# NoahVl/Explaining-In-Style-Reproducibility-Study

Measured on AMD Instinct MI355X. Metric: StylEx G+D+enc train-step images/sec @256px, higher is better.
Workload: dtype bf16; 1 GPU; FFHQ-shaped 256x256 StylEx, batch 32/GPU, GAE=2 (noise+encoder micro-steps), GP every 4th step, ResNet-18 classifier; image_size=256, batch_per_gpu=32, start_step=0, gradient_accumulate_every=2, global_batch=32, parallelism=dp1

## Files before the change

### explaining-in-style-reproducibility-study_amd/csrc/conv_igemm.hip

```cpp
#include <hip/hip_runtime.h>
#include <stdint.h>

#include "stylex_internal.h"

typedef float f32x16 __attribute__((ext_vector_type(16)));
typedef short bf16x8 __attribute__((ext_vector_type(8)));

namespace {

constexpr int BK = 32;

typedef __bf16 bf16x2_t __attribute__((ext_vector_type(2)));
typedef float f32x2_t __attribute__((ext_vector_type(2)));
__device__ __forceinline__ unsigned pack_bf16(float lo, float hi) {
    f32x2_t v = {lo, hi};
    bf16x2_t r = __builtin_convertvector(v, bf16x2_t);
    return *reinterpret_cast<unsigned*>(&r);
}
__device__ __forceinline__ unsigned short f2bf(float f) { return (unsigned short)(pack_bf16(f, 0.f) & 0xffffu); }

struct RowPix {
    int b, oh, ow;
    bool valid;
};
// ... 544 lines not shown
#pragma unroll
                for (int i = 0; i < TN_; ++i)
                    av[i] = *reinterpret_cast<const bf16x8*>(a + (wn * TN_ * 32 + i * 32 + li) * LDHA + ks * 16 + lk * 8);
#pragma unroll
                for (int j = 0; j < TC_; ++j)
                    bv[j] = *reinterpret_cast<const bf16x8*>(b + (wc * TC_ * 32 + j * 32 + li) * LDHB + ks * 16 + lk * 8);
#pragma unroll
                for (int i = 0; i < TN_; ++i)
#pragma unroll
                    for (int j = 0; j < TC_; ++j)
                        acc[i][j] = __builtin_amdgcn_mfma_f32_32x32x16_bf16(av[i], bv[j], acc[i][j], 0, 0, 0);
            }
        } else {
            const float* a = As(st) + wn * TN_ * 32 + li;
            const float* b = Bs(st) + wc * TC_ * 32 + li;
#pragma unroll
            for (int ks = 0; ks < BK / 2; ++ks) {
                float av[TN_], bv[TC_];
#pragma unroll
                for (int i = 0; i < TN_; ++i) av[i] = a[(ks * 2 + lk) * LDA + i * 32];
#pragma unroll
                for (int j = 0; j < TC_; ++j) bv[j] = b[(ks * 2 + lk) * LDB + j * 32];
#pragma unroll
                for (int i = 0; i < TN_; ++i)
#pragma unroll
                    for (int j = 0; j < TC_; ++j)
                        acc[i][j] = __builtin_amdgcn_mfma_f32_32x32x2f32(av[i], bv[j], acc[i][j], 0, 0, 0);
            }
        }
    };

    if (nk > 0) {
        load_tile(0);
        store_tile(0);
    }
    __syncthreads();
    for (int kt = 0, st = 0; kt < nk; ++kt, st ^= 1) {
        if (kt + 1 < nk) load_tile(kt + 1);
        compute(st);
        if (kt + 1 < nk) store_tile(st ^ 1);
        __syncthreads();
    }

    const int lj = lane & 31, lh = lane >> 5;
    float* out = p.y + (long)split * p.N * T * p.Ck;
#pragma unroll
    for (int j = 0; j < TC_; ++j) {
        int c = c0 + wc * TC_ * 32 + j * 32 + lj;
        if (c >= p.Ck) continue;
#pragma unroll
        for (int i = 0; i < TN_; ++i)
#pragma unroll
            for (int r = 0; r < 16; ++r) {
                int n = n0 + wn * TN_ * 32 + i * 32 + (r & 3) + 8 * (r >> 2) + 4 * lh;
                if (n < p.N) out[((long)n * T + tap) * p.Ck + c] = acc[i][j][r];
            }
    }
}

__device__ __forceinline__ float wg_out(float sum, float old, float scale, int acc) {
#pragma clang fp contract(off)
    float v = scale * sum;
    asm volatile("" : "+v"(v));
    return acc ? old + v : v;
}

__device__ __forceinline__ void bias_reduce_block(const float* __restrict__ part, float* __restrict__ db, int N, int splits,
                                                  int blk, float scale, int acc) {
    const int w = threadIdx.x >> 6, l = threadIdx.x & 63;
    const int n = blk * 4 + w;
    if (n >= N) return;
    float v = 0.f;
    for (int s = l; s < splits; s += 64) v += part[(long)s * N + n];
#pragma unroll
    for (int off = 32; off > 0; off >>= 1) v += __shfl_down(v, off);
    if (l == 0) db[n] = wg_out(v, acc ? db[n] : 0.f, scale, acc);
}

__global__ __launch_bounds__(256) void wgrad_reduce_kernel(const float* __restrict__ partial, float* dw,
                                                           int N, int C, int T, int splits, int main_blocks,
                                                           const float* __restrict__ bias_part, float* db, float scale, int accum) {
    __shared__ float tile[256 * 9];
    if ((int)blockIdx.x >= main_blocks) {
        bias_reduce_block(bias_part, db, N, splits, blockIdx.x - main_blocks, scale, accum);
        return;
    }
    const long total = (long)N * C * T;
    const long pairs = (long)N * C;
    const long i0 = (long)blockIdx.x * 256;
    const long i = i0 + threadIdx.x;
    if (T == 9) {
        float acc[9];
#pragma unroll
        for (int t = 0; t < 9; ++t) acc[t] = 0.f;
        if (i < pairs) {
            const int c = (int)(i % C);
            const long n = i / C;
            const float* src = partial + (n * 9) * C + c;
            int k = 0;
            for (; k + 4 <= splits; k += 4) {
                float v[4][9];
#pragma unroll
                for (int u = 0; u < 4; ++u)
#pragma unroll
                    for (int t = 0; t < 9; ++t) v[u][t] = src[(long)(k + u) * total + (long)t * C];
#pragma unroll
                for (int u = 0; u < 4; ++u)
#pragma unroll
                    for (int t = 0; t < 9; ++t) acc[t] += v[u][t];
            }
            for (; k < splits; ++k) {
#pragma unroll
                for (int t = 0; t < 9; ++t) acc[t] += src[(long)k * total + (long)t * C];
            }
        }
#pragma unroll
        for (int t = 0; t < 9; ++t) tile[threadIdx.x * 9 + t] = acc[t];
        __syncthreads();
        const long span = min((long)256, pairs - i0) * 9;
#pragma unroll
        for (int j = 0; j < 9; ++j) {
            const int o = j * 256 + threadIdx.x;
            if (o < span) dw[i0 * 9 + o] = wg_out(tile[o], accum ? dw[i0 * 9 + o] : 0.f, scale, accum);
        }
        return;
    }
    if (i >= pairs) return;
    const int c = (int)(i % C);
    const long n = i / C;
    const float* src = partial + (n * T) * C + c;
    float* dst = dw + i * T;
    for (int t = 0; t < T; ++t) {
        float a = 0.f;
        for (int k = 0; k < splits; ++k) a += src[(long)k * total + (long)t * C];
        dst[t] = wg_out(a, accum ? dst[t] : 0.f, scale, accum);
    }
}

template <int PP, int G>
__global__ __launch_bounds__(256) void wgrad_reduce_small_kernel(const float* __restrict__ partial, float* dw,
                                                                 int N, int C, int T, int splits, int main_blocks,
                                                                 const float* __restrict__ bias_part, float* db, float scale, int accum) {
    static_assert(PP * G == 256, "one thread per (pair, slice group)");
    __shared__ float red[G][PP][9];
    if ((int)blockIdx.x >= main_blocks) {
        bias_reduce_block(bias_part, db, N, splits, blockIdx.x - main_blocks, scale, accum);
        return;
    }
    const long total = (long)N * C * T;
    const long pairs = (long)N * C;
    const int p = threadIdx.x % PP, g = threadIdx.x / PP;
    const long i = (long)blockIdx.x * PP + p;
    const bool ok = i < pairs;
    float acc[9];
#pragma unroll
    for (int t = 0; t < 9; ++t) acc[t] = 0.f;
    if (ok) {
        const float* src = partial + ((i / C) * T) * C + (int)(i % C);
        int k = g;
        for (; k + 3 * G < splits; k += 4 * G) {
            float v[4][9];
#pragma unroll
            for (int u = 0; u < 4; ++u)
#pragma unroll
                for (int t = 0; t < 9; ++t)
                    if (t < T) v[u][t] = src[(long)(k + u * G) * total + (long)t * C];
#pragma unroll
            for (int u = 0; u < 4; ++u)
#pragma unroll
                for (int t = 0; t < 9; ++t)
                    if (t < T) acc[t] += v[u][t];
        }
        for (; k < splits; k += G) {
#pragma unroll
            for (int t = 0; t < 9; ++t)
                if (t < T) acc[t] += src[(long)k * total + (long)t * C];
        }
    }
#pragma unroll
    for (int t = 0; t < 9; ++t) red[g][p][t] = acc[t];
    __syncthreads();
    for (int o = threadIdx.x; o < PP * T; o += 256) {
        const int pp = o / T, t = o - pp * T;
        if ((long)blockIdx.x * PP + pp < pairs) {
            float sum = 0.f;
#pragma unroll
            for (int q = 0; q < G; ++q) sum += red[q][pp][t];
            float* d = dw + (long)blockIdx.x * PP * T + o;
            *d = wg_out(sum, accum ? *d : 0.f, scale, accum);
        }
    }
}

struct WgOut {
    float scale;
    int accumulate;
};
static WgOut wg_out_of(const ConvKParams& p) { return WgOut{p.wg_scale != 0.f ? p.wg_scale : 1.f, p.wg_accumulate}; }

static void launch_wgrad_reduce(const float* partial, float* dw, int N, int C, int T, int splits, hipStream_t s, WgOut wo,
                                const float* bias_part = nullptr, float* db = nullptr) {
    const long pairs = (long)N * C;
    const unsigned extra = (bias_part && db) ? (unsigned)((N + 3) / 4) : 0u;
    if (T <= 9 && splits >= 32 && (pairs <= 2048 || (pairs <= 8192 && splits >= 256))) {
        const unsigned mb = (unsigned)((pairs + 7) / 8);
        hipLaunchKernelGGL((wgrad_reduce_small_kernel<8, 32>), dim3(mb + extra), dim3(256), 0, s, partial, dw, N, C, T, splits,
                           (int)mb, bias_part, db, wo.scale, wo.accumulate);
    } else if (T <= 9 && splits >= 16 && pairs <= 16384) {
        const unsigned mb = (unsigned)((pairs + 31) / 32);
        hipLaunchKernelGGL((wgrad_reduce_small_kernel<32, 8>), dim3(mb + extra), dim3(256), 0, s, partial, dw, N, C, T, splits,
                           (int)mb, bias_part, db, wo.scale, wo.accumulate);
    } else {
        const unsigned mb = (unsigned)((pairs + 255) / 256);
        hipLaunchKernelGGL(wgrad_reduce_kernel, dim3(mb + extra), dim3(256), 0, s, partial, dw, N, C, T, splits, (int)mb,
                           bias_part, db, wo.scale, wo.accumulate);
    }
}

template <typename OUT>
__device__ __forceinline__ OUT cvt_out(float v);
template <>
__device__ __forceinline__ float cvt_out<float>(float v) { return v; }
template <>
__device__ __forceinline__ unsigned short cvt_out<unsigned short>(float v) { return f2bf(v); }

template <typename OUT>
__global__ void pack_weight_kernel(const float* __restrict__ w, OUT* __restrict__ wf, OUT* __restrict__ wb, int N,
                                   int C, int T) {
    long total = (long)N * C * T;
// ... 218 lines not shown
    int blocks = (int)(((vec4 ? total / 4 : total) + 255) / 256);
    if (blocks > 2048) blocks = 2048;
    if (vec4)
        hipLaunchKernelGGL(splitk_epilogue_kernel<true>, dim3(blocks), dim3(256), 0, s, p);
    else
        hipLaunchKernelGGL(splitk_epilogue_kernel<false>, dim3(blocks), dim3(256), 0, s, p);
    return (int)hipGetLastError();
}

int stylex_launch_igemm(ConvKParams p, int precision, void* workspace, int64_t workspace_bytes, hipStream_t s) {
    bool vec = igemm_vec_ok(p);
    if (precision == STYLEX_BF16 && !p.transposed) {
        int rc = stylex_launch_rgb(p, s);
        if (rc != STYLEX_NOT_APPLICABLE) return rc;
        rc = stylex_launch_halo(p, s);
        if (rc != STYLEX_NOT_APPLICABLE) return rc;
    }
    if (p.mask || p.gate_mask) return STYLEX_EINVAL;
    p.ksplit = 1;
    p.kt_per_split = 0;
    p.partial = nullptr;
    if (precision == STYLEX_BF16) {
        int rc = stylex_launch_gather(p, workspace, workspace_bytes, s);
        if (rc == 0) return p.ksplit ? launch_splitk_epilogue(p, s) : 0;
        if (rc != STYLEX_NOT_APPLICABLE) return rc;
    }
    if (workspace) {
        int ks, per;
        igemm_splitk_plan(p, vec, precision, &ks, &per);
        if (ks > 1 && workspace_bytes >= (int64_t)ks * p.M * p.N * (int64_t)sizeof(float)) {
            p.ksplit = ks;
            p.kt_per_split = per;
            p.partial = (float*)workspace;
        }
    }
    int rc;
    if (precision == STYLEX_BF16) {
        const int bk = igemm_bk(p, vec, precision);
        if (bk == 64) rc = dispatch_igemm<true, true, 64, true>(p, s);
        else if (bk == 33) rc = dispatch_igemm<true, true, 32, true>(p, s);
        else rc = vec ? dispatch_igemm<true, true, 32>(p, s) : dispatch_igemm<false, true, 32>(p, s);
    } else {
        rc = vec ? dispatch_igemm<true, false, 32>(p, s) : dispatch_igemm<false, false, 32>(p, s);
    }
    if (rc || p.ksplit <= 1) return rc;
    return launch_splitk_epilogue(p, s);
}

void stylex_wgrad_plan(const ConvKParams& p, int* tn, int* tc, int* splits, long* split_len) {
    bool big = p.N > 64 && p.Ck > 64;
    *tn = big ? 2 : 1;
    *tc = big ? 2 : 1;
    int bt = big ? 128 : 64;
    long tiles = (long)((p.N + bt - 1) / bt) * ((p.Ck + bt - 1) / bt) * p.KH * p.KW;
    long want = (1024 + tiles - 1) / tiles;
    long max_by_len = ((long)p.M + 4 * BK - 1) / (4 * BK);
    long sp = want < 1 ? 1 : want;
    if (sp > max_by_len) sp = max_by_len;
    if (sp < 1) sp = 1;
    if (sp > 1024) sp = 1024;
    long len = (((long)p.M + sp - 1) / sp + BK - 1) / BK * BK;
    sp = ((long)p.M + len - 1) / len;
    *splits = (int)sp;
    *split_len = len;
}

int stylex_launch_wgrad(ConvKParams p, float* partial, float* dw_oihw, int precision, hipStream_t s, float* db, int* db_done) {
    if (db_done) *db_done = 0;
    if (precision == STYLEX_BF16 && !p.s2d_c && stylex_wgrad_pipe_applicable(p)) {
        int slices = 0, tps, blocks, bias_done = 0;
        stylex_wgrad_pipe_plan(p, &slices, &tps, &blocks);
        if (db) p.bias_partial = partial + (long)slices * p.N * 9 * p.Ck;
        int rc = stylex_launch_wgrad_pipe(p, partial, s, &slices, &bias_done);
        if (rc != STYLEX_NOT_APPLICABLE) {
            if (rc) return rc;
            const bool with_db = db && bias_done;
            launch_wgrad_reduce(partial, dw_oihw, p.N, p.Ck, 9, slices, s, wg_out_of(p), with_db ? p.bias_partial : nullptr, with_db ? db : nullptr);
            if (with_db && db_done) *db_done = 1;
            return (int)hipGetLastError();
        }
        p.bias_partial = nullptr;
    }
    if (precision == STYLEX_BF16 && stylex_wgrad_tr_applicable(p)) {
        int ts = 0;
        int rc = stylex_launch_wgrad_tr(p, partial, s, &ts);
        if (rc) return rc;
        launch_wgrad_reduce(partial, dw_oihw, p.N, p.Ck, p.KH * p.KW, ts, s, wg_out_of(p));
        return (int)hipGetLastError();
    }
    int tn, tc, splits;
    long split_len;
    stylex_wgrad_plan(p, &tn, &tc, &splits, &split_len);
    p.split_len = split_len;
    p.y = partial;
    int bt = tn == 2 ? 128 : 64;
    int T = p.KH * p.KW;
    int blocks = ((p.N + bt - 1) / bt) * ((p.Ck + bt - 1) / bt) * T * splits;
    bool vec = (p.Ck % 4 == 0) && (p.N % 4 == 0) && ((reinterpret_cast<uintptr_t>(p.a) & 15) == 0) &&
               ((reinterpret_cast<uintptr_t>(p.a2) & 15) == 0) &&
               (!p.a_scale || (reinterpret_cast<uintptr_t>(p.a_scale) & 15) == 0) &&
               (!p.a2_scale || (reinterpret_cast<uintptr_t>(p.a2_scale) & 15) == 0);
    int rc;
    bool bf = precision == STYLEX_BF16;
    if (tn == 2) {
        rc = bf ? (vec ? launch_wgrad<2, 2, true, true>(p, blocks, s) : launch_wgrad<2, 2, false, true>(p, blocks, s))
                : (vec ? launch_wgrad<2, 2, true, false>(p, blocks, s) : launch_wgrad<2, 2, false, false>(p, blocks, s));
    } else {
        rc = bf ? (vec ? launch_wgrad<1, 1, true, true>(p, blocks, s) : launch_wgrad<1, 1, false, true>(p, blocks, s))
                : (vec ? launch_wgrad<1, 1, true, false>(p, blocks, s) : launch_wgrad<1, 1, false, false>(p, blocks, s));
    }
    if (rc) return rc;
    launch_wgrad_reduce(partial, dw_oihw, p.N, p.Ck, T, splits, s, wg_out_of(p));
    return (int)hipGetLastError();
}

int stylex_launch_wgrad_s2d_folded(ConvKParams p, float* partial, float* dw_oihw, hipStream_t s) {
    int slices = 0;
    int rc = stylex_launch_wgrad_pipe(p, partial, s, &slices, nullptr);
    if (rc) return rc == STYLEX_NOT_APPLICABLE ? STYLEX_EINVAL : rc;
    launch_wgrad_reduce(partial, dw_oihw, p.N, p.s2d_c, 9, slices, s, wg_out_of(p));
    return (int)hipGetLastError();
}

int stylex_launch_pack(const float* w, void* wf, void* wb, int N, int C, int T, int dtype, hipStream_t s) {
    long total = (long)N * C * T;
    int blocks = (int)((total + 255) / 256);
    if (blocks > 4096) blocks = 4096;
    if (blocks < 1) blocks = 1;
    if (dtype == STYLEX_BF16)
        hipLaunchKernelGGL(pack_weight_kernel<unsigned short>, dim3(blocks), dim3(256), 0, s, w, (unsigned short*)wf,
                           (unsigned short*)wb, N, C, T);
    else
        hipLaunchKernelGGL(pack_weight_kernel<float>, dim3(blocks), dim3(256), 0, s, w, (float*)wf, (float*)wb, N, C, T);
    return (int)hipGetLastError();
}

int stylex_launch_pack_s2d(const float* w, void* wf, void* wb, int N, int C, hipStream_t s) {
    long total = (long)N * C * 36;
    int blocks = (int)((total + 255) / 256);
    if (blocks > 4096) blocks = 4096;
    hipLaunchKernelGGL(pack_weight_s2d_kernel, dim3(blocks), dim3(256), 0, s, w, (unsigned short*)wf, (unsigned short*)wb, N, C);
    return (int)hipGetLastError();
}

int stylex_launch_fold_s2d(const float* dw2, float* dw, int N, int C, hipStream_t s) {
    long total = (long)N * C * 9;
    int blocks = (int)((total + 255) / 256);
    if (blocks > 4096) blocks = 4096;
    hipLaunchKernelGGL(fold_weight_s2d_kernel, dim3(blocks), dim3(256), 0, s, dw2, dw, N, C);
    return (int)hipGetLastError();
}
```

### explaining-in-style-reproducibility-study_amd/csrc/conv_wgrad_pipe.hip

```cpp
#include <hip/hip_runtime.h>
#include <stdint.h>
#include <stdlib.h>

#include "stylex_internal.h"

typedef float f32x16 __attribute__((ext_vector_type(16)));
typedef short bf16x8 __attribute__((ext_vector_type(8)));
typedef short s16x4 __attribute__((ext_vector_type(4)));

struct StylexWgPipeArgs {
    int total_tiles;
    int tiles_per_split;
    int otiles, c_tiles;
    int tx_count, ty_count;
};

namespace {

typedef StylexWgPipeArgs WgArgs;
typedef __attribute__((address_space(3))) void* lds_void_ptr;

template <int NP64, int TW>
struct WgCfg {
    static constexpr int kTW = TW;
// ... 47 lines not shown

constexpr unsigned WG_ALL_TAPS = 0x1ffu;
constexpr bool wg_kw_used(unsigned mask, int kw) { return ((mask >> kw) | (mask >> (3 + kw)) | (mask >> (6 + kw))) & 1u; }

template <class Cfg, int S, unsigned MASK = WG_ALL_TAPS>
__device__ __forceinline__ void issue_reads(WgOps& o, const int (&xb)[4], int dyb) {
    constexpr int rho = S % (Cfg::RW + 2), pw = S / (Cfg::RW + 2), par = S & 1;
    static_assert(Cfg::HWD % 4 == 2, "swizzle class of a halo pixel");
    constexpr int q0 = (rho * Cfg::HWD + pw * 16 + 0) * 128, q1 = (rho * Cfg::HWD + pw * 16 + 1) * 128,
                  q2 = (rho * Cfg::HWD + pw * 16 + 2) * 128;
    constexpr int m0 = (2 * rho + 0) & 3, m1 = (2 * rho + 1) & 3, m2 = (2 * rho + 2) & 3;
    if constexpr (wg_kw_used(MASK, 0)) {
        tr_read<q0>(o.b[par][0][0], xb[m0]);
        tr_read<q0 + 512>(o.b[par][0][1], xb[m0]);
    }
    if constexpr (wg_kw_used(MASK, 1)) {
        tr_read<q1>(o.b[par][1][0], xb[m1]);
        tr_read<q1 + 512>(o.b[par][1][1], xb[m1]);
    }
    if constexpr (wg_kw_used(MASK, 2)) {
        tr_read<q2>(o.b[par][2][0], xb[m2]);
        tr_read<q2 + 512>(o.b[par][2][1], xb[m2]);
    }
    if constexpr (rho < Cfg::RW) {
        constexpr int qa = (rho * Cfg::kTW + pw * 16) * 128;
        tr_read<qa>(o.a[rho & 3][0], dyb);
        tr_read<qa + 512>(o.a[rho & 3][1], dyb);
    }
}

template <class Cfg, int S>
__device__ __forceinline__ void wait_reads(WgOps& o) {
    constexpr int rho = S % (Cfg::RW + 2), par = S & 1;
    if constexpr (rho < Cfg::RW)
        asm volatile("s_waitcnt lgkmcnt(0)"
                     : "+v"(o.b[par][0][0]), "+v"(o.b[par][0][1]), "+v"(o.b[par][1][0]), "+v"(o.b[par][1][1]),
                       "+v"(o.b[par][2][0]), "+v"(o.b[par][2][1]), "+v"(o.a[rho & 3][0]), "+v"(o.a[rho & 3][1]));
    else
        asm volatile("s_waitcnt lgkmcnt(0)"
                     : "+v"(o.b[par][0][0]), "+v"(o.b[par][0][1]), "+v"(o.b[par][1][0]), "+v"(o.b[par][1][1]),
                       "+v"(o.b[par][2][0]), "+v"(o.b[par][2][1]));
}

template <class Cfg, int S, bool BIAS, unsigned MASK = WG_ALL_TAPS>
__device__ __forceinline__ void step_mfma(f32x16 (&acc)[9], f32x16& accb, const WgOps& o, bool do_bias, const bf16x8& ones) {
    constexpr int rho = S % (Cfg::RW + 2), par = S & 1;
    const bf16x8 b0 = cat8(o.b[par][0][0], o.b[par][0][1]);
    const bf16x8 b1 = cat8(o.b[par][1][0], o.b[par][1][1]);
    const bf16x8 b2 = cat8(o.b[par][2][0], o.b[par][2][1]);
#pragma unroll
    for (int kh = 0; kh < 3; ++kh) {
        const int r = rho - kh;
        if (r >= 0 && r < Cfg::RW) {
            const bf16x8 av = cat8(o.a[r & 3][0], o.a[r & 3][1]);
            if ((MASK >> (kh * 3 + 0)) & 1u) mfma1(acc[kh * 3 + 0], av, b0);
            if ((MASK >> (kh * 3 + 1)) & 1u) mfma1(acc[kh * 3 + 1], av, b1);
            if ((MASK >> (kh * 3 + 2)) & 1u) mfma1(acc[kh * 3 + 2], av, b2);
        }
    }
    if constexpr (BIAS && rho < Cfg::RW) {
        if (do_bias) {
            const bf16x8 av = cat8(o.a[rho & 3][0], o.a[rho & 3][1]);
            mfma1(accb, av, ones);
        }
    }
}

constexpr unsigned WG_OOB = 0x80000000u;

struct WgCursor {
    int t, b, tx, ty;
};

template <int NP64, int TW, bool BIAS, bool S2D = false>
__global__ __launch_bounds__(512, 2) void conv3x3_wgrad_pipe_kernel(ConvKParams p, WgArgs wa) {
    using Cfg = WgCfg<NP64, TW>;
    constexpr int TR = Cfg::TR, HWD = Cfg::HWD, XPX = Cfg::XPX, X_PIECES = Cfg::X_PIECES;
    constexpr int X_STRIDE = Cfg::X_STRIDE, DY_STRIDE = Cfg::DY_STRIDE, DY_BASE = Cfg::DY_BASE;
    constexpr int XS = Cfg::XS, DS = Cfg::DS, NSLOT = Cfg::NSLOT, NSTEP = Cfg::NSTEP, NX = Cfg::NX, ND = Cfg::ND;
    constexpr int XA = Cfg::XA, DA = Cfg::DA, WAITN = Cfg::WAITN;
    static_assert(NSTEP % 2 == 0, "the operand ping-pong restarts at parity 0 every stage");
    static_assert(NSLOT <= 2 * (NSTEP - 1), "at most two DMA pieces per step");
    static_assert(XA <= DA, "issue order inside a stage: the one-ahead stream first");
    static_assert(!(S2D && BIAS), "the space-to-depth path has no bias sums");
    extern __shared__ __attribute__((aligned(16))) char smem[];
    const int tid = threadIdx.x, lane = tid & 63;
    const int wave = __builtin_amdgcn_readfirstlane(tid >> 6);
    const int W = p.Wo, C = p.Ck, N = p.N;

    int bid = blockIdx.x;
    {
        const int nblk = gridDim.x, q = nblk >> 3, rr = nblk & 7, xcd = bid & 7, idx = bid >> 3;
        bid = (xcd < rr ? xcd * (q + 1) : rr * (q + 1) + (xcd - rr) * q) + idx;
    }
    const int split = __builtin_amdgcn_readfirstlane(bid / wa.otiles);
    const int ot = bid - split * wa.otiles;
    const int nt_ = __builtin_amdgcn_readfirstlane(ot / wa.c_tiles);
    const int n0 = nt_ * (64 * NP64), c0 = (ot - nt_ * wa.c_tiles) * 64;
    const int t_begin = split * wa.tiles_per_split;
    const int t_end = min(wa.total_tiles, t_begin + wa.tiles_per_split);
    const int nst = t_end - t_begin;
    if (nst <= 0) return;

    const int cblk = wave & 1, nb4 = wave >> 1;
    const int nhalf = nb4 & 1, hi2 = nb4 >> 1;
    const int dy_wave_off = NP64 == 2 ? hi2 * 16384 : (TW == 32 ? hi2 * 16 * 128 : hi2 * 4 * TW * 128);
    const int x_wave_off = NP64 == 2 ? 0 : (TW == 32 ? hi2 * 16 * 128 : hi2 * 4 * HWD * 128);

    const int i16 = lane & 15, g = lane >> 4;
    const int lane_px = ((g >> 1) * 8 + (i16 >> 2)) * 128 + (g & 1) * 32 + (i16 & 3) * 8;
    int dyb = lane_px + ((nhalf ^ ((i16 >> 3) & 1)) * 64) + dy_wave_off + DY_BASE;
    int xb[4];
#pragma unroll
    for (int m = 0; m < 4; ++m) xb[m] = lane_px + ((cblk ^ (((m + (i16 >> 2)) >> 1) & 1)) * 64) + x_wave_off;

    const int dpx = lane >> 3;
    const unsigned lslot = (unsigned)((lane & 7) ^ (((lane >> 4) & 1) << 2));
    unsigned vxc[XS];
    int xdst[XS];
#pragma unroll
    for (int k = 0; k < XS; ++k) {
        const int piece = wave + 8 * k;
        const int q = piece * 8 + dpx;
        const int row = q / HWD, col = q - row * HWD;
        const bool ok = piece < X_PIECES && q < XPX && c0 + (int)lslot * 8 < C;
        const unsigned edge = (row == 0 ? 1u : 0u) | (row == TR + 1 ? 2u : 0u) | (col == 0 ? 4u : 0u) | (col == TW + 1 ? 8u : 0u);
        vxc[k] = ok ? (((unsigned)(row * W + col) * (unsigned)C + (unsigned)c0 + lslot * 8u) * 2u) | edge : WG_OOB;
        xdst[k] = piece < X_PIECES ? piece * 1024 : -1;
    }
    unsigned vdy[DS];
#pragma unroll
    for (int k = 0; k < DS; ++k) {
        const int piece = wave + 8 * k;
        const int q = (piece & 15) * 8 + dpx;
        const int r = q / TW, col = q - r * TW;
        const int nch = n0 + (piece >> 4) * 64 + (int)lslot * 8;
        vdy[k] = nch < N ? ((unsigned)(r * W + col) * (unsigned)N + (unsigned)nch) * 2u : WG_OOB;
    }
    const int Hs = __builtin_amdgcn_readfirstlane(p.Ho), Ws = __builtin_amdgcn_readfirstlane(p.Wo);
    const int Cs = __builtin_amdgcn_readfirstlane(p.Ck), Ns = __builtin_amdgcn_readfirstlane(p.N);
    const uint64_t xbase = reinterpret_cast<uint64_t>(p.a) - (uint64_t)((long)(Ws + 1) * Cs * 2);
    const uint64_t xbase_u = ((uint64_t)(unsigned)__builtin_amdgcn_readfirstlane((int)(xbase >> 32)) << 32) |
                             (unsigned)__builtin_amdgcn_readfirstlane((int)(xbase & 0xffffffffu));
    const __amdgpu_buffer_rsrc_t rx = __builtin_amdgcn_make_buffer_rsrc(reinterpret_cast<void*>(xbase_u), 0, 0x40000000, 0x00020000);
    const __amdgpu_buffer_rsrc_t rdy = __builtin_amdgcn_make_buffer_rsrc(const_cast<float*>(p.a2), 0, 0x40000000, 0x00020000);

    WgCursor cx, cd;
    {
        const int r1 = __builtin_amdgcn_readfirstlane(t_begin / wa.ty_count);
        const int b1 = __builtin_amdgcn_readfirstlane(r1 / wa.tx_count);
        cx.t = t_begin, cx.ty = t_begin - r1 * wa.ty_count, cx.tx = r1 - b1 * wa.tx_count, cx.b = b1;
        cd = cx;
    }
    auto advance = [&](WgCursor& c) {
        ++c.t;
        if (++c.ty == wa.ty_count) {
            c.ty = 0;
            if (++c.tx == wa.tx_count) c.tx = 0, ++c.b;
        }
    };
    int xslot_dma = 0, dslot_dma = 0;
#define WG_ISSUE_X(K)                                                                                                \
    {                                                                                                                \
        const bool more_ = cx.t < t_end;                                                                             \
        const unsigned soff_ = (unsigned)(((cx.b * Hs + cx.ty * TR) * Ws + cx.tx * TW) * Cs) * 2u;                   \
        const unsigned edge_ = (cx.ty == 0 ? 1u : 0u) | (cx.ty == wa.ty_count - 1 ? 2u : 0u) | (cx.tx == 0 ? 4u : 0u) | \
                               (cx.tx == wa.tx_count - 1 ? 8u : 0u);                                                 \
// ... 86 lines not shown
            WG_STEP(2)                                    \
            WG_STEP(3)                                    \
            WG_STEP(4)                                    \
            if constexpr (NSTEP == 6) {                   \
                WG_LAST(5)                                \
            } else {                                      \
                WG_STEP(5)                                \
                WG_STEP(6)                                \
                WG_STEP(7)                                \
                WG_STEP(8)                                \
                if constexpr (NSTEP == 12) {              \
                    WG_STEP(9)                            \
                    WG_STEP(10)                           \
                    WG_LAST(11)                           \
                } else {                                  \
                    WG_LAST(9)                            \
                }                                         \
            }                                             \
        }                                                 \
    }
    const int sub = S2D ? c0 / p.s2d_c : 0;
    if constexpr (!S2D) {
        WG_LOOP(WG_ALL_TAPS)
    } else {
        if (sub == 0) WG_LOOP(0x010u)
        else if (sub == 1) WG_LOOP(0x018u)
        else if (sub == 2) WG_LOOP(0x012u)
        else WG_LOOP(0x01bu)
    }
#undef WG_LOOP
#undef WG_LAST
#undef WG_STEP
#undef WG_ISSUE
#undef WG_END_DY
#undef WG_END_X
#undef WG_ISSUE_DY
#undef WG_ISSUE_X
    asm volatile("s_waitcnt lgkmcnt(0)" ::: "memory");
    wait_vmcnt<0>();

    asm volatile("s_nop 15\n\ts_nop 15"
                 : "+v"(acc[0]), "+v"(acc[1]), "+v"(acc[2]), "+v"(acc[3]), "+v"(acc[4]), "+v"(acc[5]), "+v"(acc[6]),
                   "+v"(acc[7]), "+v"(acc[8]), "+v"(accb));

    if constexpr (NP64 == 1) {
        float4* cb = reinterpret_cast<float4*>(smem) + (wave & 3) * (5 * 4 * 64) + lane;
#pragma unroll
        for (int round = 0; round < 2; ++round) {
            __syncthreads();
            if (hi2 == 1) {
#pragma unroll
                for (int tt = 0; tt < 5; ++tt) {
                    const int t = round * 5 + tt;
#pragma unroll
                    for (int q = 0; q < 4; ++q) {
                        const f32x16& v = t < 9 ? acc[t < 9 ? t : 0] : accb;
                        cb[(tt * 4 + q) * 64] = make_float4(v[4 * q], v[4 * q + 1], v[4 * q + 2], v[4 * q + 3]);
                    }
                }
            }
            __syncthreads();
            if (hi2 == 0) {
#pragma unroll
                for (int tt = 0; tt < 5; ++tt) {
                    const int t = round * 5 + tt;
#pragma unroll
                    for (int q = 0; q < 4; ++q) {
                        const float4 u = cb[(tt * 4 + q) * 64];
                        f32x16& v = t < 9 ? acc[t < 9 ? t : 0] : accb;
                        v[4 * q] += u.x, v[4 * q + 1] += u.y, v[4 * q + 2] += u.z, v[4 * q + 3] += u.w;
                    }
                }
            }
        }
        if (hi2 == 1) return;
    }

    const int nbase = n0 + (NP64 == 2 ? nb4 : nhalf) * 32;
    const int lj = lane & 31, lh = lane >> 5;
    if constexpr (S2D) {
        const int Co = p.s2d_c, sy = sub >> 1, sx = sub & 1;
        float* outf = p.y + (long)split * N * 9 * Co;
        const int cl = c0 - sub * Co + cblk * 32 + lj;
#pragma unroll
        for (int t2 = 0; t2 < 5; ++t2) {
            if (t2 == 2) continue;
            const int kh2 = t2 / 3, kw2 = t2 % 3;
            if ((kh2 == 0 && sy == 0) || (kw2 == 0 && sx == 0)) continue;
            const int tap = (kh2 == 0 ? 0 : sy + 1) * 3 + (kw2 == 0 ? 0 : sx + 1);
#pragma unroll
            for (int r = 0; r < 16; ++r) {
                const int n = nbase + (r & 3) + 8 * (r >> 2) + 4 * lh;
                outf[((long)n * 9 + tap) * Co + cl] = acc[t2][r];
            }
        }
        return;
    }
    float* out = p.y + (long)split * N * 9 * C;
    const int c = c0 + cblk * 32 + lj;
    if (nbase >= N || c0 + cblk * 32 >= C) return;
    if (do_bias && lj == 0) {
#pragma unroll
        for (int r = 0; r < 16; ++r) p.bias_partial[(long)split * N + nbase + (r & 3) + 8 * (r >> 2) + 4 * lh] = accb[r];
    }
    if (c >= C) return;
    const float xsc = p.a_scale ? p.a_scale[(long)(t_begin / (wa.tx_count * wa.ty_count)) * C + c] : 1.f;
#pragma unroll
    for (int t = 0; t < 9; ++t)
#pragma unroll
        for (int r = 0; r < 16; ++r) {
            const int n = nbase + (r & 3) + 8 * (r >> 2) + 4 * lh;
            out[((long)n * 9 + t) * C + c] = acc[t][r] * xsc;
        }
}

template <int NP64, int TW>
int launch_wg_s2d(const ConvKParams& p, const WgArgs& wa, int blocks, hipStream_t s) {
    using Cfg = WgCfg<NP64, TW>;
    static int attr_state = 0;
    if (attr_state == 0) {
        hipError_t e = hipFuncSetAttribute(reinterpret_cast<const void*>(conv3x3_wgrad_pipe_kernel<NP64, TW, false, true>),
                                           hipFuncAttributeMaxDynamicSharedMemorySize, Cfg::SMEM);
        attr_state = e == hipSuccess ? 1 : -1;
    }
    if (attr_state < 0) return STYLEX_NOT_APPLICABLE;
    stylex_note_kernel("conv3x3_wgrad_pipe_kernel<%d, %d, false, true>", NP64, TW);
    hipLaunchKernelGGL((conv3x3_wgrad_pipe_kernel<NP64, TW, false, true>), dim3(blocks), dim3(512), Cfg::SMEM, s, p, wa);
    return (int)hipGetLastError();
}

template <int NP64, int TW>
int launch_wg(const ConvKParams& p, const WgArgs& wa, int blocks, bool bias, hipStream_t s) {
    using Cfg = WgCfg<NP64, TW>;
    static bool attr_done = false;
    if (!attr_done) {
        hipError_t e = hipFuncSetAttribute(reinterpret_cast<const void*>(conv3x3_wgrad_pipe_kernel<NP64, TW, true>),
                                           hipFuncAttributeMaxDynamicSharedMemorySize, Cfg::SMEM);
        if (e != hipSuccess) return STYLEX_NOT_APPLICABLE;
        e = hipFuncSetAttribute(reinterpret_cast<const void*>(conv3x3_wgrad_pipe_kernel<NP64, TW, false>),
                                hipFuncAttributeMaxDynamicSharedMemorySize, Cfg::SMEM);
        if (e != hipSuccess) return STYLEX_NOT_APPLICABLE;
        attr_done = true;
    }
    stylex_note_kernel("conv3x3_wgrad_pipe_kernel<%d, %d, %s, false>", NP64, TW, bias ? "true" : "false");
    if (bias) hipLaunchKernelGGL((conv3x3_wgrad_pipe_kernel<NP64, TW, true>), dim3(blocks), dim3(512), Cfg::SMEM, s, p, wa);
    else hipLaunchKernelGGL((conv3x3_wgrad_pipe_kernel<NP64, TW, false>), dim3(blocks), dim3(512), Cfg::SMEM, s, p, wa);
    return (int)hipGetLastError();
}

int g_wg_cus = 0;

}

static int wg_np64(const ConvKParams& p) {
    const char* env = getenv("STYLEX_WGRAD_PIPE_NP");
    if (p.N % 128 != 0 || (env && env[0] == '1')) return 1;
    if (env && env[0] == '2') return 2;
    const int tw = p.Wo >= 32 ? 32 : 16;
    const long tiles = (long)p.B * (p.Wo / tw) * (p.Ho / (128 / tw));
    const long otiles2 = (long)(p.N / 128) * ((p.Ck + 63) / 64);
    const long cus = g_wg_cus > 0 ? g_wg_cus : 256;
    const long per_block = tiles * otiles2 / cus;
    static const long thr = getenv("STYLEX_WGRAD_PIPE_NP_THR") ? atol(getenv("STYLEX_WGRAD_PIPE_NP_THR")) : 48;
    return per_block < thr ? 1 : 2;
}

bool stylex_wgrad_pipe_applicable(const ConvKParams& p) {
    const char* env = getenv("STYLEX_WGRAD_PIPE");
    if (env && env[0] == '0') return false;
    if (!p.act_bf16 || p.KH != 3 || p.KW != 3 || p.stride != 1 || p.pad != 1 || p.Hi != p.Ho || p.Wi != p.Wo) return false;
    if (p.a2_scale) return false;
    if (p.s2d_c && (p.Ck != 4 * p.s2d_c || p.s2d_c % 64 != 0 || p.N % 64 != 0 || p.a_scale)) return false;
    if ((p.Ck % 64 != 0 && p.Ck != 32) || (p.N % 64 != 0 && p.N != 32)) return false;
    const int tw = p.Wo >= 32 ? 32 : 16;
    if (p.Wo % tw != 0 || p.Wo < 16) return false;
    const int tr = 128 / tw;
    if (p.Ho % tr != 0) return false;
    if ((reinterpret_cast<uintptr_t>(p.a) & 15) || (reinterpret_cast<uintptr_t>(p.a2) & 15)) return false;
    if (p.a_scale && (reinterpret_cast<uintptr_t>(p.a_scale) & 3)) return false;
    if ((long)p.B * p.Ho * p.Wo * p.Ck * 2 >= (1l << 30) + (1l << 29) || (long)p.B * p.Ho * p.Wo * p.N * 2 >= (1l << 30) + (1l << 29))
        return false;
    return true;
}

void stylex_wgrad_pipe_plan(const ConvKParams& p, int* slices, int* tiles_per_split, int* blocks) {
    if (!g_wg_cus) {
        int dev = 0, n = 0;
        if (hipGetDevice(&dev) == hipSuccess) (void)hipDeviceGetAttribute(&n, hipDeviceAttributeMultiprocessorCount, dev);
        g_wg_cus = n > 0 ? n : 256;
    }
    const int np64 = wg_np64(p);
    const int tw = p.Wo >= 32 ? 32 : 16;
    const int tr = 128 / tw;
    const long tiles_img = (long)(p.Wo / tw) * (p.Ho / tr);
    const long tiles = (long)p.B * tiles_img;
    const long otiles = (long)((p.N + 64 * np64 - 1) / (64 * np64)) * ((p.Ck + 63) / 64);
    long want = g_wg_cus / otiles;
    if (want < 1) want = 1;
    if (want > tiles) want = tiles;
    long tps = (tiles + want - 1) / want;
    if (p.a_scale) {
        if (tps > tiles_img) tps = tiles_img;
        while (tiles_img % tps) --tps;
    }
    const long splits = (tiles + tps - 1) / tps;
    *tiles_per_split = (int)tps;
    *blocks = (int)(splits * otiles);
    *slices = (int)splits;
}

int stylex_launch_wgrad_pipe(ConvKParams p, float* partial, hipStream_t s, int* slices_out, int* bias_done) {
    if (!stylex_wgrad_pipe_applicable(p)) return STYLEX_NOT_APPLICABLE;
    int slices, tps, blocks;
    stylex_wgrad_pipe_plan(p, &slices, &tps, &blocks);
    const int np64 = wg_np64(p);
    const int tw = p.Wo >= 32 ? 32 : 16;
    const int tr = 128 / tw;
    WgArgs wa;
    wa.tx_count = p.Wo / tw;
    wa.ty_count = p.Ho / tr;
    wa.total_tiles = p.B * wa.tx_count * wa.ty_count;
    wa.tiles_per_split = tps;
    wa.c_tiles = (p.Ck + 63) / 64;
    wa.otiles = ((p.N + 64 * np64 - 1) / (64 * np64)) * wa.c_tiles;
    p.y = partial;
    *slices_out = slices;
    if (p.s2d_c) {
        if (bias_done) *bias_done = 0;
        p.bias_partial = nullptr;
        if (np64 == 2) return tw == 32 ? launch_wg_s2d<2, 32>(p, wa, blocks, s) : launch_wg_s2d<2, 16>(p, wa, blocks, s);
        return tw == 32 ? launch_wg_s2d<1, 32>(p, wa, blocks, s) : launch_wg_s2d<1, 16>(p, wa, blocks, s);
    }
    const bool bias = p.bias_partial != nullptr;
    if (bias_done) *bias_done = bias ? 1 : 0;
    if (np64 == 2) return tw == 32 ? launch_wg<2, 32>(p, wa, blocks, bias, s) : launch_wg<2, 16>(p, wa, blocks, bias, s);
    return tw == 32 ? launch_wg<1, 32>(p, wa, blocks, bias, s) : launch_wg<1, 16>(p, wa, blocks, bias, s);
}
```

### explaining-in-style-reproducibility-study_amd/csrc/conv_wgrad_tr.hip

```cpp
#include <hip/hip_runtime.h>
#include <stdint.h>
#include <stdlib.h>

#include "stylex_internal.h"

typedef float f32x16 __attribute__((ext_vector_type(16)));
typedef short bf16x8 __attribute__((ext_vector_type(8)));
typedef short s16x4 __attribute__((ext_vector_type(4)));
typedef __bf16 bf16x2_t __attribute__((ext_vector_type(2)));
typedef float f32x2_t __attribute__((ext_vector_type(2)));

namespace {

__device__ __forceinline__ unsigned pack_bf16(float lo, float hi) {
    f32x2_t v = {lo, hi};
    bf16x2_t r = __builtin_convertvector(v, bf16x2_t);
    return *reinterpret_cast<unsigned*>(&r);
}

typedef __attribute__((address_space(3))) s16x4* lds_s4_ptr;

__device__ __forceinline__ bf16x8 tr_read8(const char* base, int byte_off) {
    s16x4 lo = __builtin_amdgcn_ds_read_tr16_b64_v4i16((lds_s4_ptr)(base + byte_off));
    s16x4 hi = __builtin_amdgcn_ds_read_tr16_b64_v4i16((lds_s4_ptr)(base + byte_off + 4 * 64));
// ... 25 lines not shown
    const int N = p.N, C = p.Ck;
    const int n_tiles = (N + BNn - 1) / BNn, c_tiles = C8 ? 1 : (C + BC - 1) / BC;
    const int per_split = n_tiles * c_tiles * Teff;

    const int bid = blockIdx.x;
    const int tile = bid % per_split, split = bid / per_split;
    const int tap = tile % Teff;
    const int n0 = ((tile / Teff) / c_tiles) * BNn;
    const int c0 = ((tile / Teff) % c_tiles) * BC;
    const int kh = tap / p.KW, kw = tap - kh * p.KW;

    const int m_begin = (int)((long)split * p.split_len);
    const int m_end = (int)min((long)p.M, (long)m_begin + p.split_len);
    const int nk = (m_end - m_begin + BKP - 1) / BKP;
    const int hw = p.Ho * p.Wo;
    const bool pow2 = (hw & (hw - 1)) == 0 && (p.Wo & (p.Wo - 1)) == 0;
    const int sh_hw = __builtin_ctz((unsigned)hw), sh_w = __builtin_ctz((unsigned)p.Wo);

    constexpr int A_SLOTS = BNn / 8, B_SLOTS = BC / 8;
    constexpr int A_PER = BKP * A_SLOTS / 256, B_PER = BKP * B_SLOTS / 256;
    uint4 ra[A_PER], rb[B_PER];
    const unsigned short* dy = reinterpret_cast<const unsigned short*>(p.a2);
    const unsigned short* xs = reinterpret_cast<const unsigned short*>(p.a);

    auto scaled = [&](uint4 v, const float* sc) -> uint4 {
        float4 a0 = *reinterpret_cast<const float4*>(sc), a1 = *reinterpret_cast<const float4*>(sc + 4);
        float4 f0 = act_unpack4(make_uint2(v.x, v.y)), f1 = act_unpack4(make_uint2(v.z, v.w));
        v.x = pack_bf16(f0.x * a0.x, f0.y * a0.y); v.y = pack_bf16(f0.z * a0.z, f0.w * a0.w);
        v.z = pack_bf16(f1.x * a1.x, f1.y * a1.y); v.w = pack_bf16(f1.z * a1.z, f1.w * a1.w);
        return v;
    };

    auto load_tile = [&](int kt) {
        const int mb = m_begin + kt * BKP;
#pragma unroll
        for (int j = 0; j < A_PER; ++j) {
            const int idx = tid + 256 * j;
            const int pr = idx / A_SLOTS, q = idx % A_SLOTS;
            const int m = mb + pr;
            const int n = n0 + q * 8;
            uint4 v = make_uint4(0u, 0u, 0u, 0u);
            if (m < m_end && n < N) {
                v = *reinterpret_cast<const uint4*>(dy + (long)m * N + n);
                if (p.a2_scale) v = scaled(v, p.a2_scale + (long)(pow2 ? (unsigned)m >> sh_hw : (unsigned)m / (unsigned)hw) * N + n);
            }
            ra[j] = v;
        }
#pragma unroll
        for (int j = 0; j < B_PER; ++j) {
            const int idx = tid + 256 * j;
            const int pr = idx / B_SLOTS, q = idx % B_SLOTS;
            const int m = mb + pr;
            int c, th, tw;
            bool ok = m < m_end;
            if (C8) {
                c = 0;
                th = q / p.KW;
                tw = q - th * p.KW;
                ok = ok && q < T;
            } else {
                c = c0 + q * 8;
                th = kh;
                tw = kw;
                ok = ok && c < C;
            }
            uint4 v = make_uint4(0u, 0u, 0u, 0u);
            if (ok) {
                int b, oh;
                if (pow2) {
                    b = (int)((unsigned)m >> sh_hw);
                    oh = (int)(((unsigned)m & (unsigned)(hw - 1)) >> sh_w);
                } else {
                    b = (int)((unsigned)m / (unsigned)hw);
                    oh = (int)((unsigned)(m - b * hw) / (unsigned)p.Wo);
                }
                const int r = m - b * hw;
                const int ow = r - oh * p.Wo;
                const int ih = oh * p.stride + th - p.pad, iw = ow * p.stride + tw - p.pad;
                if (ih >= 0 && ih < p.Hi && iw >= 0 && iw < p.Wi) {
                    v = *reinterpret_cast<const uint4*>(xs + (((long)b * p.Hi + ih) * p.Wi + iw) * C + c);
                    if (p.a_scale) v = scaled(v, p.a_scale + (long)b * C + c);
                }
            }
            rb[j] = v;
        }
    };

    auto store_tile = [&](int st) {
        char* base = smem + st * STAGE;
#pragma unroll
        for (int j = 0; j < A_PER; ++j) {
            const int idx = tid + 256 * j;
            const int pr = idx / A_SLOTS, q = idx % A_SLOTS;
            *reinterpret_cast<uint4*>(base + (q >> 2) * PANEL + pr * 64 + (q & 3) * 16) = ra[j];
        }
#pragma unroll
        for (int j = 0; j < B_PER; ++j) {
            const int idx = tid + 256 * j;
            const int pr = idx / B_SLOTS, q = idx % B_SLOTS;
            *reinterpret_cast<uint4*>(base + (NPA + (q >> 2)) * PANEL + pr * 64 + (q & 3) * 16) = rb[j];
        }
    };

    f32x16 acc[TN_][TC_];
#pragma unroll
    for (int i = 0; i < TN_; ++i)
#pragma unroll
        for (int j = 0; j < TC_; ++j)
#pragma unroll
            for (int e = 0; e < 16; ++e) acc[i][j][e] = 0.f;

    const int i16 = lane & 15, g = lane >> 4;
    const int lane_off = ((g >> 1) * 8 + (i16 >> 2)) * 64 + ((g & 1) * 16 + (i16 & 3) * 4) * 2;

    auto compute = [&](int st) {
        const char* a_base = smem + st * STAGE + (wn * TN_) * PANEL + lane_off;
        const char* b_base = smem + st * STAGE + (NPA + wc * TC_) * PANEL + lane_off;
#pragma unroll
        for (int ks = 0; ks < BKP / 16; ++ks) {
            bf16x8 av[TN_], bv[TC_];
#pragma unroll
            for (int i = 0; i < TN_; ++i) av[i] = tr_read8(a_base + i * PANEL, ks * 16 * 64);
#pragma unroll
            for (int j = 0; j < TC_; ++j) bv[j] = tr_read8(b_base + j * PANEL, ks * 16 * 64);
#pragma unroll
            for (int i = 0; i < TN_; ++i)
#pragma unroll
                for (int j = 0; j < TC_; ++j)
                    acc[i][j] = __builtin_amdgcn_mfma_f32_32x32x16_bf16(av[i], bv[j], acc[i][j], 0, 0, 0);
        }
    };

    if (nk > 0) {
        load_tile(0);
        store_tile(0);
    }
    __syncthreads();
    for (int kt = 0, st = 0; kt < nk; ++kt, st ^= 1) {
        if (kt + 1 < nk) load_tile(kt + 1);
        compute(st);
        if (kt + 1 < nk) store_tile(st ^ 1);
        __syncthreads();
    }

    const int lj = lane & 31, lh = lane >> 5;
    float* out = p.y + (long)split * N * T * C;
#pragma unroll
    for (int j = 0; j < TC_; ++j) {
        const int cj = c0 + (wc * TC_ + j) * 32 + lj;
        if (C8 ? (cj >= T * 8) : (cj >= C)) continue;
#pragma unroll
        for (int i = 0; i < TN_; ++i)
#pragma unroll
            for (int r = 0; r < 16; ++r) {
                const int n = n0 + (wn * TN_ + i) * 32 + (r & 3) + 8 * (r >> 2) + 4 * lh;
                if (n < N) out[C8 ? ((long)n * T * 8 + cj) : (((long)n * T + tap) * C + cj)] = acc[i][j][r];
            }
    }
}

constexpr int DSTAGES = 4, DPIECES = 4;
constexpr int DSTAGE_BYTES = 8 * PANEL;

struct TrOps {
    s16x4 a[2];
    s16x4 b[2][2];
};
template <int OFF>
__device__ __forceinline__ void tr_asm(s16x4& dst, int addr) {
    asm volatile("ds_read_b64_tr_b16 %0, %1 offset:%2" : "=v"(dst) : "v"(addr), "n"(OFF));
}
template <int KS>
__device__ __forceinline__ void tr_issue(TrOps& o, int a_addr, int b_addr) {
    tr_asm<KS * 16 * 64>(o.a[0], a_addr);
    tr_asm<KS * 16 * 64 + 4 * 64>(o.a[1], a_addr);
    tr_asm<KS * 16 * 64>(o.b[0][0], b_addr);
    tr_asm<KS * 16 * 64 + 4 * 64>(o.b[0][1], b_addr);
    tr_asm<PANEL + KS * 16 * 64>(o.b[1][0], b_addr);
    tr_asm<PANEL + KS * 16 * 64 + 4 * 64>(o.b[1][1], b_addr);
}
template <int N>
__device__ __forceinline__ void tr_wait(TrOps& o) {
    asm volatile("s_waitcnt lgkmcnt(%6)"
                 : "+v"(o.a[0]), "+v"(o.a[1]), "+v"(o.b[0][0]), "+v"(o.b[0][1]), "+v"(o.b[1][0]), "+v"(o.b[1][1])
                 : "n"(N));
}
__device__ __forceinline__ bf16x8 cat8(s16x4 lo, s16x4 hi) {
    bf16x8 r;
    r[0] = lo[0]; r[1] = lo[1]; r[2] = lo[2]; r[3] = lo[3];
    r[4] = hi[0]; r[5] = hi[1]; r[6] = hi[2]; r[7] = hi[3];
    return r;
}

__global__ __launch_bounds__(512, 1) void conv_wgrad_tr_dma_kernel(ConvKParams p) {
    extern __shared__ __attribute__((aligned(16))) char smem[];
    const int tid = threadIdx.x, lane = tid & 63;
    const int wave = __builtin_amdgcn_readfirstlane(tid >> 6);
    const int T = p.KH * p.KW;
    const int N = __builtin_amdgcn_readfirstlane(p.N), C = __builtin_amdgcn_readfirstlane(p.Ck);
    const int n_tiles = N >> 7, c_tiles = C >> 7;
    const int per_split = n_tiles * c_tiles * T;
    const int bid = blockIdx.x;
    const int tile = bid % per_split, split = bid / per_split;
    const int tap = tile % T;
    const int n0 = ((tile / T) / c_tiles) << 7;
    const int c0 = ((tile / T) % c_tiles) << 7;
    const int kh = tap / p.KW, kw = tap - kh * p.KW;
    const int m_begin = (int)((long)split * p.split_len);
    const int m_end = (int)min((long)p.M, (long)m_begin + p.split_len);
    const int nk = (m_end - m_begin + BKP - 1) / BKP;
    const int Wo = __builtin_amdgcn_readfirstlane(p.Wo), hw = __builtin_amdgcn_readfirstlane(p.Ho * p.Wo);
    const int Hi = __builtin_amdgcn_readfirstlane(p.Hi), Wi = __builtin_amdgcn_readfirstlane(p.Wi);
    const int sh_hw = __builtin_ctz((unsigned)hw), sh_w = __builtin_ctz((unsigned)Wo);
    const int dh = kh - p.pad, dw = kw - p.pad, strd = __builtin_amdgcn_readfirstlane(p.stride);

    const __amdgpu_buffer_rsrc_t rdy = __builtin_amdgcn_make_buffer_rsrc(const_cast<float*>(p.a2), 0, 0x7ffffff0, 0x00020000);
    const __amdgpu_buffer_rsrc_t rx = __builtin_amdgcn_make_buffer_rsrc(const_cast<float*>(p.a), 0, 0x7ffffff0, 0x00020000);
    constexpr unsigned OOBV = 0x80000000u;
    typedef __attribute__((address_space(3))) void* lds_void_ptr;

    const bool stage_x = wave >= 4;
    const int panel = wave & 3;
    const int chan = panel * 32 + (lane & 3) * 8;
    int mrow[DPIECES];
    unsigned a_off[DPIECES];
#pragma unroll
    for (int it = 0; it < DPIECES; ++it) {
        mrow[it] = m_begin + it * 16 + (lane >> 2);
        a_off[it] = ((unsigned)mrow[it] * (unsigned)N + (unsigned)(n0 + chan)) * 2u;
    }
    int i_kt = 0;
    auto issue_stage = [&](int rs) {
        const int dst = rs * DSTAGE_BYTES + ((stage_x ? 4 : 0) + panel) * PANEL;
        const int mshift = i_kt * BKP;
        if (!stage_x) {
            const unsigned soff = (unsigned)mshift * (unsigned)N * 2u;
#pragma unroll
            for (int it = 0; it < DPIECES; ++it) {
                const unsigned v = mrow[it] + mshift < m_end ? a_off[it] : OOBV;
                __builtin_amdgcn_raw_ptr_buffer_load_lds(rdy, (lds_void_ptr)(smem + dst + it * 1024), 16, v, soff, 0, 0);
            }
        } else {
#pragma unroll
            for (int it = 0; it < DPIECES; ++it) {
                const int m = mrow[it] + mshift;
                const int b = (int)((unsigned)m >> sh_hw), r = m & (hw - 1);
                const int ih = (r >> sh_w) * strd + dh, iw = (r & (Wo - 1)) * strd + dw;
                const bool ok = m < m_end && (unsigned)ih < (unsigned)Hi && (unsigned)iw < (unsigned)Wi;
                const unsigned v = ok ? ((unsigned)((b * Hi + ih) * Wi + iw) * (unsigned)C + (unsigned)(c0 + chan)) * 2u : OOBV;
                __builtin_amdgcn_raw_ptr_buffer_load_lds(rx, (lds_void_ptr)(smem + dst + it * 1024), 16, v, 0u, 0, 0);
            }
        }
        ++i_kt;
    };

    const int wn = wave >> 1, wc = wave & 1;
    f32x16 acc[2];
#pragma unroll
    for (int j = 0; j < 2; ++j)
#pragma unroll
        for (int e = 0; e < 16; ++e) acc[j][e] = 0.f;
    const int i16 = lane & 15, g = lane >> 4;
    const int lane_off = ((g >> 1) * 8 + (i16 >> 2)) * 64 + ((g & 1) * 16 + (i16 & 3) * 4) * 2;
    const int lds0 = (int)(unsigned)(uintptr_t)(lds_void_ptr)smem;

    for (int s = 0; s < 3 && s < nk; ++s) issue_stage(s);
    for (int kt = 0; kt < nk; ++kt) {
        if (kt + 2 < nk) asm volatile("s_waitcnt vmcnt(%0)" ::"n"(2 * DPIECES) : "memory");
        else if (kt + 1 < nk) asm volatile("s_waitcnt vmcnt(%0)" ::"n"(DPIECES) : "memory");
        else asm volatile("s_waitcnt vmcnt(0)" ::: "memory");
        asm volatile("s_waitcnt lgkmcnt(0)" ::: "memory");
        __builtin_amdgcn_s_barrier();
        asm volatile("" ::: "memory");
        if (kt + 3 < nk) issue_stage((kt + 3) % DSTAGES);
        const int a_addr = lds0 + (kt % DSTAGES) * DSTAGE_BYTES + wn * PANEL + lane_off;
        const int b_addr = lds0 + (kt % DSTAGES) * DSTAGE_BYTES + (4 + wc * 2) * PANEL + lane_off;
        TrOps o[2];
        tr_issue<0>(o[0], a_addr, b_addr);
#pragma unroll
        for (int ks = 0; ks < BKP / 16; ++ks) {
            if (ks + 1 < BKP / 16) {
                if (ks == 0) tr_issue<1>(o[1], a_addr, b_addr);
                if (ks == 1) tr_issue<2>(o[0], a_addr, b_addr);
                if (ks == 2) tr_issue<3>(o[1], a_addr, b_addr);
                tr_wait<6>(o[ks & 1]);
            } else {
                tr_wait<0>(o[ks & 1]);
            }
            const bf16x8 av = cat8(o[ks & 1].a[0], o[ks & 1].a[1]);
            acc[0] = __builtin_amdgcn_mfma_f32_32x32x16_bf16(av, cat8(o[ks & 1].b[0][0], o[ks & 1].b[0][1]), acc[0], 0, 0, 0);
            acc[1] = __builtin_amdgcn_mfma_f32_32x32x16_bf16(av, cat8(o[ks & 1].b[1][0], o[ks & 1].b[1][1]), acc[1], 0, 0, 0);
        }
    }

    const int lj = lane & 31, lh = lane >> 5;
    float* out = p.y + (long)split * N * T * C;
#pragma unroll
    for (int j = 0; j < 2; ++j) {
        const int cj = c0 + (wc * 2 + j) * 32 + lj;
#pragma unroll
        for (int r = 0; r < 16; ++r) {
            const int n = n0 + wn * 32 + (r & 3) + 8 * (r >> 2) + 4 * lh;
            out[((long)n * T + tap) * C + cj] = acc[j][r];
        }
    }
}

static bool tr_dma_applicable(const ConvKParams& p) {
    const char* env = getenv("STYLEX_WGRAD_TR_DMA");
    if (env && env[0] == '0') return false;
    const int hw = p.Ho * p.Wo;
    if (!p.act_bf16 || p.a_scale || p.a2_scale || p.s2d_c) return false;
    if (!((p.KH == 3 && p.KW == 3 && p.pad == 1) || (p.KH == 1 && p.KW == 1 && p.pad == 0))) return false;
    if (!((p.stride == 1 && p.Hi == p.Ho && p.Wi == p.Wo) || (p.stride == 2 && p.KH == 3 && p.Hi == 2 * p.Ho && p.Wi == 2 * p.Wo))) return false;
    if (p.N % 128 != 0 || p.Ck % 128 != 0 || (hw & (hw - 1)) || (p.Wo & (p.Wo - 1))) return false;
    if (hw > 64 && p.KH != 1) return false;
    if ((long)p.M * p.N * 2 >= (1l << 31) - 16 || (long)p.M * p.Ck * 2 >= (1l << 31) - 16) return false;
    return true;
}

template <int TN_, int TC_, bool C8>
int launch_tr(const ConvKParams& p, int blocks, hipStream_t s) {
    auto k = conv_wgrad_tr_kernel<TN_, TC_, C8>;
    constexpr int smem_bytes = TrGeom<TN_, TC_>::SMEM_BYTES;
    static bool attr_done = false;
    if (!attr_done) {
        hipError_t e = hipFuncSetAttribute(reinterpret_cast<const void*>(k), hipFuncAttributeMaxDynamicSharedMemorySize,
                                           smem_bytes);
        if (e != hipSuccess) return (int)e;
        attr_done = true;
    }
    stylex_note_kernel("conv_wgrad_tr_kernel<%d, %d, %s>", TN_, TC_, C8 ? "true" : "false");
    hipLaunchKernelGGL(k, dim3(blocks), dim3(256), smem_bytes, s, p);
    return (int)hipGetLastError();
}

}

bool stylex_wgrad_tr_applicable(const ConvKParams& p) {
    if (!p.act_bf16 || p.Ck % 8 != 0 || p.N % 8 != 0 || p.s2d_c) return false;
    if ((reinterpret_cast<uintptr_t>(p.a) & 15) || (reinterpret_cast<uintptr_t>(p.a2) & 15)) return false;
    if (p.a_scale && (reinterpret_cast<uintptr_t>(p.a_scale) & 15)) return false;
    if (p.a2_scale && (reinterpret_cast<uintptr_t>(p.a2_scale) & 15)) return false;
    if (p.Ck == 8 && p.KH * p.KW > 16) return false;
    return true;
}

void stylex_wgrad_tr_plan(const ConvKParams& p, int* mode, int* splits, long* split_len) {
    const int T = p.KH * p.KW;
    long tiles;
    if (p.Ck == 8) {
        *mode = 2;
        tiles = (p.N + 63) / 64;
    } else if (p.N > 64 && p.Ck > 64) {
        *mode = 0;
        tiles = (long)((p.N + 127) / 128) * ((p.Ck + 127) / 128) * T;
    } else {
        *mode = 1;
        tiles = (long)((p.N + 63) / 64) * ((p.Ck + 63) / 64) * T;
    }
    const bool dma = *mode == 0 && tr_dma_applicable(p);
    long want = ((dma ? 384 : 768) + tiles - 1) / tiles;
    long max_by_len = ((long)p.M + (dma ? 8 : 2) * BKP - 1) / ((dma ? 8 : 2) * BKP);
    long sp = want < 1 ? 1 : want;
    if (sp > max_by_len) sp = max_by_len;
    if (sp < 1) sp = 1;
    if (sp > 1024) sp = 1024;
    long len = (((long)p.M + sp - 1) / sp + BKP - 1) / BKP * BKP;
    sp = ((long)p.M + len - 1) / len;
    *splits = (int)sp;
    *split_len = len;
}

int stylex_launch_wgrad_tr(ConvKParams p, float* partial, hipStream_t s, int* splits_out) {
    int mode, splits;
    long len;
    stylex_wgrad_tr_plan(p, &mode, &splits, &len);
    p.split_len = len;
    p.y = partial;
    *splits_out = splits;
    const int T = p.KH * p.KW;
    if (mode == 2) return launch_tr<1, 2, true>(p, ((p.N + 63) / 64) * splits, s);
    if (mode == 0 && tr_dma_applicable(p)) {
        static bool attr_done = false;
        if (!attr_done) {
            hipError_t e = hipFuncSetAttribute(reinterpret_cast<const void*>(conv_wgrad_tr_dma_kernel),
                                               hipFuncAttributeMaxDynamicSharedMemorySize, DSTAGES * DSTAGE_BYTES);
            if (e != hipSuccess) return (int)e;
            attr_done = true;
        }
        stylex_note_kernel("conv_wgrad_tr_dma_kernel");
        hipLaunchKernelGGL(conv_wgrad_tr_dma_kernel, dim3((p.N / 128) * (p.Ck / 128) * T * splits), dim3(512), DSTAGES * DSTAGE_BYTES, s, p);
        return (int)hipGetLastError();
    }
    if (mode == 0) return launch_tr<2, 2, false>(p, ((p.N + 127) / 128) * ((p.Ck + 127) / 128) * T * splits, s);
    return launch_tr<1, 1, false>(p, ((p.N + 63) / 64) * ((p.Ck + 63) / 64) * T * splits, s);
}
```

### explaining-in-style-reproducibility-study_amd/csrc/stylex_capi.hip

```cpp
#include <hip/hip_runtime.h>
#include <stdint.h>
#include <stdarg.h>
#include <stdio.h>
#include <string.h>

#include <array>
#include <map>
#include <mutex>
#include <string>
#include <vector>

#include "stylex_internal.h"

namespace {

typedef std::array<int64_t, 9> LayerKey;
struct TimedLaunch {
    hipEvent_t start, stop;
    int cls;
    double flops;
    double bytes;
    LayerKey key;
    char kernel[112];
};
// ... 328 lines not shown
    ConvKParams p;
    if (int rc = s2d_res_params(p, sh, s2d_c, res_c)) return rc;
    p.a = (const float*)x_s2d;
    p.w = w_fwd_s2d;
    p.y = (float*)y;
    p.bias = bias;
    p.x2 = x_res;
    p.w2 = w_res;
    p.res_scale = scale;
    const double flops = 2.0 * p.M * (double)p.N * (p.Ck * 9 / 4.0 + p.c2);
    ScopedTimer tm(0, flops, conv_bytes(sh, STYLEX_BF16_ACT, false) + 2.0 * p.M * p.c2, (hipStream_t)stream, sh, p.s2d_c);
    const int rc = stylex_launch_halo_dma(p, (hipStream_t)stream);
    return rc == STYLEX_NOT_APPLICABLE ? STYLEX_EINVAL : rc;
}

int stylex_conv2d_bwd_data(const void* dy, const void* w_bwd, void* dx, const int64_t* sh, int flags,
                           const stylex_conv_epilogue* epi, int precision, void* workspace, int64_t workspace_bytes,
                           void* stream) {
    if (!dy || !w_bwd || !dx || !conv_shape_ok(sh) || sh[7] > 2) return STYLEX_EINVAL;
    if (precision != STYLEX_F32 && precision != STYLEX_BF16 && precision != STYLEX_BF16_ACT) return STYLEX_EINVAL;
    if (flags & ~(STYLEX_EPI_OSCALE | STYLEX_EPI_GATE | STYLEX_EPI_GATE_MASK)) return STYLEX_EINVAL;
    if ((flags & STYLEX_EPI_GATE) && (!epi || !epi->residual)) return STYLEX_EINVAL;
    if ((flags & STYLEX_EPI_GATE_MASK) && ((flags & STYLEX_EPI_GATE) || !epi || !epi->mask || precision != STYLEX_BF16_ACT))
        return STYLEX_EINVAL;
    ConvKParams p;
    bwd_data_params(p, sh);
    p.a = (const float*)dy;
    p.w = w_bwd;
    p.y = (float*)dx;
    p.act_bf16 = precision == STYLEX_BF16_ACT;
    if (p.act_bf16) precision = STYLEX_BF16;
    if (precision == STYLEX_BF16 && p.KH == 3 && p.stride == 1 && p.pad == 1) {
        ConvKParams q = p;
        q.flip_taps = 1;
        q.flags = flags;
        if (epi) {
            q.a_scale = epi->in_scale;
            q.out_scale = epi->out_scale;
            q.residual = (const float*)epi->residual;
            q.res_scale = epi->res_scale;
            q.s2d_c = (int)epi->s2d_c;
            if (flags & STYLEX_EPI_GATE_MASK) q.gate_mask = (const unsigned char*)epi->mask;
            if (q.s2d_c && (q.N != 4 * q.s2d_c || q.s2d_c % 64)) return STYLEX_EINVAL;
        }
        if (!((flags & STYLEX_EPI_OSCALE) && !q.out_scale)) {
            double fl = 2.0 * (double)sh[0] * sh[9] * sh[10] * (double)sh[4] * sh[3] * sh[5] * sh[6] / (q.s2d_c ? 4.0 : 1.0);
            ScopedTimer tmh(1, fl, conv_bytes(sh, q.act_bf16 ? STYLEX_BF16_ACT : precision, false), (hipStream_t)stream, sh, q.s2d_c);
            int rc = stylex_launch_halo(q, (hipStream_t)stream);
            if (rc != STYLEX_NOT_APPLICABLE) return rc;
            if (tmh.on) {
                (void)hipEventDestroy(tmh.t.start);
                (void)hipEventDestroy(tmh.t.stop);
                tmh.on = false;
            }
        }
    }
    if (flags & STYLEX_EPI_GATE_MASK) return STYLEX_EINVAL;
    p.transposed = 1;
    p.phase_major = (p.stride == 2 && (p.Ho % 2 == 0) && (p.Wo % 2 == 0)) ? 1 : 0;
    p.flags = flags;
    if (epi) {
        p.a_scale = epi->in_scale;
        p.out_scale = epi->out_scale;
        p.residual = (const float*)epi->residual;
        p.res_scale = epi->res_scale;
    }
    if ((flags & STYLEX_EPI_OSCALE) && !p.out_scale) return STYLEX_EINVAL;
    double flops = 2.0 * (double)sh[0] * sh[9] * sh[10] * (double)sh[4] * sh[3] * sh[5] * sh[6];
    ScopedTimer tm(1, flops, conv_bytes(sh, p.act_bf16 ? STYLEX_BF16_ACT : precision, false), (hipStream_t)stream, sh, 0);
    return stylex_launch_igemm(p, precision, workspace, workspace_bytes, (hipStream_t)stream);
}

static void wgrad_params(ConvKParams& p, const int64_t* sh) {
    fill_common(p, sh);
    p.Hi = (int)sh[1];
    p.Wi = (int)sh[2];
    p.Ck = (int)sh[3];
    p.N = (int)sh[4];
    p.Ho = (int)sh[9];
    p.Wo = (int)sh[10];
    p.M = p.B * p.Ho * p.Wo;
}

int64_t stylex_conv2d_bwd_weight_workspace_bytes(const int64_t* sh) {
    if (!conv_shape_ok(sh)) return STYLEX_EINVAL;
    ConvKParams p;
    wgrad_params(p, sh);
    int tn, tc, splits;
    long len;
    stylex_wgrad_plan(p, &tn, &tc, &splits, &len);
    {
        static const float dummy_scale[4] = {0.f, 0.f, 0.f, 0.f};
        for (int sc = 0; sc < 2; ++sc) {
            ConvKParams q = p;
            q.act_bf16 = 1;
            q.a = q.a2 = nullptr;
            q.a_scale = sc ? dummy_scale : nullptr;
            if (stylex_wgrad_pipe_applicable(q)) {
                int sl, tps, blocks;
                stylex_wgrad_pipe_plan(q, &sl, &tps, &blocks);
                if (sl > splits) splits = sl;
            }
        }
    }
    if (p.Ck % 8 == 0 && p.N % 8 == 0) {
        for (int abf = 0; abf < 2; ++abf) {
            ConvKParams q = p;
            q.act_bf16 = abf;
            int mode, ts;
            long tl;
            stylex_wgrad_tr_plan(q, &mode, &ts, &tl);
            if (ts > splits) splits = ts;
        }
    }
    return (int64_t)splits * p.N * p.Ck * p.KH * p.KW * (int64_t)sizeof(float) + (int64_t)splits * p.N * (int64_t)sizeof(float);
}

int stylex_conv2d_bwd_weight(const void* x, const void* dy, float* dw, void* workspace, int64_t workspace_bytes,
                             const int64_t* sh, const float* x_scale, const float* dy_scale, int s2d_c, int precision,
                             void* stream) {
    return stylex_conv2d_bwd_weight_bias(x, dy, dw, nullptr, nullptr, workspace, workspace_bytes, sh, x_scale, dy_scale, s2d_c,
                                         precision, stream);
}

int stylex_conv2d_bwd_weight_bias(const void* x, const void* dy, float* dw, float* db, int* db_written, void* workspace,
                                  int64_t workspace_bytes, const int64_t* sh, const float* x_scale, const float* dy_scale,
                                  int s2d_c, int precision, void* stream) {
    return stylex_conv2d_bwd_weight_ex(x, dy, dw, db, db_written, workspace, workspace_bytes, sh, x_scale, dy_scale, s2d_c, 1.f, 0,
                                       precision, stream);
}

int stylex_conv2d_bwd_weight_ex(const void* x, const void* dy, float* dw, float* db, int* db_written, void* workspace,
                                int64_t workspace_bytes, const int64_t* sh, const float* x_scale, const float* dy_scale,
                                int s2d_c, float out_scale, int accumulate, int precision, void* stream) {
    if (db_written) *db_written = 0;
    if (db && !db_written) return STYLEX_EINVAL;
    if (!x || !dy || !dw || !workspace || !conv_shape_ok(sh) || sh[7] > 2) return STYLEX_EINVAL;
    if (precision != STYLEX_F32 && precision != STYLEX_BF16 && precision != STYLEX_BF16_ACT) return STYLEX_EINVAL;
    if (workspace_bytes < stylex_conv2d_bwd_weight_workspace_bytes(sh)) return STYLEX_EWORKSPACE;
    ConvKParams p;
    wgrad_params(p, sh);
    p.a = (const float*)x;
    p.a_scale = x_scale;
    p.a2 = (const float*)dy;
    p.a2_scale = dy_scale;
    p.act_bf16 = precision == STYLEX_BF16_ACT;
    if (p.act_bf16) precision = STYLEX_BF16;
    p.s2d_c = s2d_c;
    p.wg_scale = out_scale;
    p.wg_accumulate = accumulate ? 1 : 0;
    if (s2d_c && (p.Ck != 4 * s2d_c || s2d_c % 64 || p.KH != 3 || p.stride != 1)) return STYLEX_EINVAL;
    double flops = 2.0 * p.M * (double)p.N * p.Ck * p.KH * p.KW / (s2d_c ? 4.0 : 1.0);
    ScopedTimer tm(2, flops, conv_bytes(sh, p.act_bf16 ? STYLEX_BF16_ACT : precision, true), (hipStream_t)stream, sh, s2d_c);
    return stylex_launch_wgrad(p, (float*)workspace, dw, precision, (hipStream_t)stream, db, db_written);
}

int stylex_conv2d_bwd_weight_s2d_supported(const int64_t* sh, int s2d_c, int precision) {
    if (!conv_shape_ok(sh) || precision != STYLEX_BF16_ACT || s2d_c <= 0) return 0;
    ConvKParams p;
    wgrad_params(p, sh);
    p.act_bf16 = 1;
    p.s2d_c = s2d_c;
    return stylex_wgrad_pipe_applicable(p) ? 1 : 0;
}

int stylex_conv2d_bwd_weight_s2d(const void* x2, const void* dy, float* dw, void* workspace, int64_t workspace_bytes,
                                 const int64_t* sh, int s2d_c, float out_scale, int accumulate, int precision, void* stream) {
    if (!x2 || !dy || !dw || !workspace || !conv_shape_ok(sh) || precision != STYLEX_BF16_ACT || s2d_c <= 0) return STYLEX_EINVAL;
    if (workspace_bytes < stylex_conv2d_bwd_weight_workspace_bytes(sh)) return STYLEX_EWORKSPACE;
    ConvKParams p;
    wgrad_params(p, sh);
    p.a = (const float*)x2;
    p.a2 = (const float*)dy;
    p.act_bf16 = 1;
    p.s2d_c = s2d_c;
    p.wg_scale = out_scale;
    p.wg_accumulate = accumulate ? 1 : 0;
    if (!stylex_wgrad_pipe_applicable(p)) return STYLEX_EINVAL;
    double flops = 2.0 * p.M * (double)p.N * p.Ck * 9 / 4.0;
    ScopedTimer tm(2, flops, conv_bytes(sh, STYLEX_BF16_ACT, true), (hipStream_t)stream, sh, s2d_c);
    return stylex_launch_wgrad_s2d_folded(p, (float*)workspace, dw, (hipStream_t)stream);
}

int stylex_pack_weight_s2d(const float* w, void* wf, void* wb, const int64_t* sh, void* stream) {
    if (!w || sh[0] < 1 || sh[1] < 1 || sh[2] != 3 || sh[3] != 3) return STYLEX_EINVAL;
    return stylex_launch_pack_s2d(w, wf, wb, (int)sh[0], (int)sh[1], (hipStream_t)stream);
}

int stylex_fold_weight_grad_s2d(const float* dw2, float* dw, const int64_t* sh, void* stream) {
    if (!dw2 || !dw || sh[0] < 1 || sh[1] < 1 || sh[2] != 3 || sh[3] != 3) return STYLEX_EINVAL;
    return stylex_launch_fold_s2d(dw2, dw, (int)sh[0], (int)sh[1], (hipStream_t)stream);
}

}
```

### explaining-in-style-reproducibility-study_amd/csrc/stylex_internal.h

```cpp
#pragma once
#include <hip/hip_runtime.h>
#include <stdint.h>

#include "../../include/stylex_hip.h"
#include "act_io.h"

struct ConvKParams {
    const float* a;
    const float* a_scale;
    const void* w;
    const float* a2;
    const float* a2_scale;
    float* y;
    const float* bias;
    const float* out_scale;
    const float* noise;
    const float* noise_w;
    const float* noise_b;
    const float* residual;
    float res_scale;
    int noise_stride;
    int B, Hi, Wi, Ck, N, KH, KW, Ho, Wo, stride, pad;
    int transposed;
    int phase_major;
    int act_bf16;
    int s2d_c;
    int flip_taps;
    int M;
    int flags;
    long split_len;
    int ksplit;
    int kt_per_split;
    float* partial;
    unsigned char* mask;
    const unsigned char* gate_mask;
    int dry;
    float* bias_partial;
    const void* x2;
    const void* w2;
    int c2;
    float wg_scale;
    int wg_accumulate;
};

int stylex_launch_igemm(ConvKParams p, int precision, void* workspace, int64_t workspace_bytes, hipStream_t s);
int64_t stylex_igemm_workspace_bytes(const ConvKParams& p, int precision);
void stylex_wgrad_plan(const ConvKParams& p, int* tn, int* tc, int* splits, long* split_len);
int stylex_launch_wgrad(ConvKParams p, float* partial, float* dw_oihw, int precision, hipStream_t s, float* db = nullptr,
                        int* db_done = nullptr);
int stylex_launch_pack(const float* w, void* wf, void* wb, int N, int C, int T, int dtype, hipStream_t s);

#define STYLEX_NOT_APPLICABLE (-100)

void stylex_note_kernel(const char* fmt, ...);
#define STYLEX_TIMING_INPUT 3
class StylexTimedCall {
  public:
    StylexTimedCall(int cls, double bytes, hipStream_t s);
    ~StylexTimedCall();
    StylexTimedCall(const StylexTimedCall&) = delete;
    StylexTimedCall& operator=(const StylexTimedCall&) = delete;

  private:
    void* impl_;
};

#ifdef __HIPCC__
__device__ __forceinline__ unsigned stylex_sign_bits8(uint4 v) {
    const unsigned w[4] = {v.x, v.y, v.z, v.w};
    unsigned m = 0;
#pragma unroll
    for (int d = 0; d < 4; ++d) {
        m |= (__uint_as_float(w[d] << 16) > 0.f ? 1u : 0u) << (2 * d);
        m |= (__uint_as_float(w[d] & 0xffff0000u) > 0.f ? 1u : 0u) << (2 * d + 1);
    }
    return m;
}
#endif
int stylex_launch_halo(const ConvKParams& p, hipStream_t s);

int stylex_launch_halo_dma(const ConvKParams& p, hipStream_t s);

int stylex_launch_rgb(const ConvKParams& p, hipStream_t s);

int stylex_launch_pipe(const ConvKParams& p, hipStream_t s);
int stylex_launch_line64(const ConvKParams& p, hipStream_t s);

int stylex_launch_s2d_dgrad(const ConvKParams& p, hipStream_t s);
int stylex_launch_s2d_fwd(const ConvKParams& p, hipStream_t s);

int stylex_launch_gather(ConvKParams& p, void* workspace, int64_t workspace_bytes, hipStream_t s);
int64_t stylex_gather_workspace_bytes(const ConvKParams& p);

bool stylex_wgrad_pipe_applicable(const ConvKParams& p);
void stylex_wgrad_pipe_plan(const ConvKParams& p, int* slices, int* tiles_per_split, int* blocks);
int stylex_launch_wgrad_pipe(ConvKParams p, float* partial, hipStream_t s, int* slices_out, int* bias_done = nullptr);
int stylex_launch_wgrad_s2d_folded(ConvKParams p, float* partial, float* dw_oihw, hipStream_t s);

bool stylex_wgrad_tr_applicable(const ConvKParams& p);
void stylex_wgrad_tr_plan(const ConvKParams& p, int* mode, int* splits, long* split_len);
int stylex_launch_wgrad_tr(ConvKParams p, float* partial, hipStream_t s, int* splits_out);

__host__ __device__ inline unsigned stylex_s2d_tap_mask(int s) {
    const int sy = s >> 1, sx = s & 1;
    unsigned m = 0;
    for (int kh = 0; kh < 2; ++kh)
        for (int kw = 0; kw < 2; ++kw)
            if ((kh == 1 || sy == 1) && (kw == 1 || sx == 1)) m |= 1u << (kh * 3 + kw);
    return m;
}
int stylex_launch_pack_s2d(const float* w, void* wf, void* wb, int N, int C, hipStream_t s);
int stylex_launch_fold_s2d(const float* dw2, float* dw, int N, int C, hipStream_t s);
```

### explaining-in-style-reproducibility-study_amd/stylex/hip_backend.py

```python
import os as _os

if _os.environ.get("STYLEX_MIOPEN_ALLOW_BWD_GTC", "0") != "1":
    _os.environ.setdefault("MIOPEN_DEBUG_CONV_IMPLICIT_GEMM_ASM_BWD_GTC_XDLOPS_NHWC", "0")

import atexit
import ctypes
import os
import weakref

import torch

_HERE = os.path.dirname(os.path.abspath(__file__))
LIB_PATH = os.path.join(os.path.dirname(_HERE), "libstylex_hip.so")

F32, BF16, BF16_ACT = 0, 1, 2
EPI_BIAS, EPI_LRELU, EPI_OSCALE, EPI_NOISE, EPI_RESIDUAL, EPI_RELU, EPI_GATE, EPI_NOISE_NAT = 1, 2, 4, 8, 16, 32, 64, 128
EPI_MASK_OUT, EPI_GATE_MASK = 256, 512

_c_f = ctypes.c_void_p
_i64p = ctypes.POINTER(ctypes.c_int64)


class ConvEpilogue(ctypes.Structure):
    _fields_ = [
        ("in_scale", ctypes.c_void_p),
        ("bias", ctypes.c_void_p),
        ("out_scale", ctypes.c_void_p),
        ("noise", ctypes.c_void_p),
        ("noise_stride", ctypes.c_int64),
        ("noise_w", ctypes.c_void_p),
        ("noise_b", ctypes.c_void_p),
        ("residual", ctypes.c_void_p),
        ("res_scale", ctypes.c_float),
        ("s2d_c", ctypes.c_int32),
        ("mask", ctypes.c_void_p),
    ]


SIGNATURES = {
    "stylex_init": (ctypes.c_int, [ctypes.c_int]),
    "stylex_version": (ctypes.c_char_p, []),
    "stylex_pack_weight": (ctypes.c_int, [_c_f, _c_f, _c_f, _i64p, ctypes.c_int, ctypes.c_void_p]),
    "stylex_conv2d_workspace_bytes": (ctypes.c_int64, [_i64p, ctypes.c_int, ctypes.c_int]),
    "stylex_conv2d_fwd": (ctypes.c_int, [_c_f, _c_f, _c_f, _i64p, ctypes.c_int, ctypes.POINTER(ConvEpilogue),
                                         ctypes.c_int, ctypes.c_void_p, ctypes.c_int64, ctypes.c_void_p]),
    "stylex_conv2d_bwd_data": (ctypes.c_int, [_c_f, _c_f, _c_f, _i64p, ctypes.c_int, ctypes.POINTER(ConvEpilogue),
                                              ctypes.c_int, ctypes.c_void_p, ctypes.c_int64, ctypes.c_void_p]),
    "stylex_conv2d_bwd_weight_workspace_bytes": (ctypes.c_int64, [_i64p]),
    "stylex_conv2d_bwd_weight": (ctypes.c_int, [_c_f, _c_f, _c_f, ctypes.c_void_p, ctypes.c_int64, _i64p, _c_f, _c_f,
                                                ctypes.c_int, ctypes.c_int, ctypes.c_void_p]),
    "stylex_conv2d_bwd_weight_bias": (ctypes.c_int, [_c_f, _c_f, _c_f, _c_f, ctypes.POINTER(ctypes.c_int), ctypes.c_void_p,
                                                     ctypes.c_int64, _i64p, _c_f, _c_f, ctypes.c_int, ctypes.c_int,
                                                     ctypes.c_void_p]),
    "stylex_conv2d_bwd_weight_ex": (ctypes.c_int, [_c_f, _c_f, _c_f, _c_f, ctypes.POINTER(ctypes.c_int), ctypes.c_void_p,
                                                   ctypes.c_int64, _i64p, _c_f, _c_f, ctypes.c_int, ctypes.c_float, ctypes.c_int,
                                                   ctypes.c_int, ctypes.c_void_p]),
    "stylex_blur3x3_s2d_fwd": (ctypes.c_int, [_c_f, _c_f, _i64p, ctypes.c_int, ctypes.c_void_p]),
    "stylex_blur3x3_s2d_bwd": (ctypes.c_int, [_c_f, _c_f, _i64p, ctypes.c_int, ctypes.c_void_p]),
    "stylex_blur3x3_reflect_bwd_gate": (ctypes.c_int, [_c_f, _c_f, ctypes.c_float, _c_f, _i64p, ctypes.c_int, ctypes.c_void_p]),
    "stylex_blur3x3_s2d_bwd_gate": (ctypes.c_int, [_c_f, _c_f, ctypes.c_float, _c_f, _i64p, ctypes.c_int, ctypes.c_void_p]),
    "stylex_blur3x3_s2d_bwd_gate_mask": (ctypes.c_int, [_c_f, _c_f, ctypes.c_float, _c_f, _i64p, ctypes.c_int, ctypes.c_void_p]),
    "stylex_conv_mask_supported": (ctypes.c_int, [_i64p, ctypes.c_int, ctypes.c_int, ctypes.c_int]),
    "stylex_add_at_even": (ctypes.c_int, [_c_f, _c_f, _i64p, ctypes.c_int, ctypes.c_void_p]),
    "stylex_subsample2_fwd": (ctypes.c_int, [_c_f, _c_f, _i64p, ctypes.c_int, ctypes.c_void_p]),
    "stylex_subsample2_bwd": (ctypes.c_int, [_c_f, _c_f, _i64p, ctypes.c_int, ctypes.c_void_p]),
    "stylex_pack_weight_s2d": (ctypes.c_int, [_c_f, _c_f, _c_f, _i64p, ctypes.c_void_p]),
    "stylex_fold_weight_grad_s2d": (ctypes.c_int, [_c_f, _c_f, _i64p, ctypes.c_void_p]),
    "stylex_conv2d_bwd_weight_s2d_supported": (ctypes.c_int, [_i64p, ctypes.c_int, ctypes.c_int]),
    "stylex_conv2d_bwd_weight_s2d": (ctypes.c_int, [ctypes.c_void_p, ctypes.c_void_p, _c_f, ctypes.c_void_p, ctypes.c_int64, _i64p,
                                                    ctypes.c_int, ctypes.c_float, ctypes.c_int, ctypes.c_int, ctypes.c_void_p]),
    "stylex_upsample2x_bilinear_fwd": (ctypes.c_int, [_c_f, _c_f, _i64p, ctypes.c_int, ctypes.c_void_p]),
    "stylex_upsample2x_bilinear_bwd": (ctypes.c_int, [_c_f, _c_f, _i64p, ctypes.c_int, ctypes.c_void_p]),
    "stylex_rgb_up_blur_add_fwd": (ctypes.c_int, [_c_f, _c_f, _c_f, _i64p, ctypes.c_int, ctypes.c_void_p]),
    "stylex_rgb_up_blur_add_bwd": (ctypes.c_int, [_c_f, _c_f, _i64p, ctypes.c_int, ctypes.c_void_p]),
    "stylex_blur3x3_reflect_fwd": (ctypes.c_int, [_c_f, _c_f, _i64p, ctypes.c_int, ctypes.c_void_p]),
    "stylex_blur3x3_reflect_bwd": (ctypes.c_int, [_c_f, _c_f, _i64p, ctypes.c_int, ctypes.c_void_p]),
    "stylex_bias_act_fwd": (ctypes.c_int, [_c_f, _c_f, _c_f, ctypes.c_int64, _c_f, _c_f, _c_f, _i64p, ctypes.c_int,
                                           ctypes.c_void_p]),
    "stylex_bias_act_bwd": (ctypes.c_int, [_c_f, _c_f, _c_f, _i64p, ctypes.c_int, ctypes.c_void_p]),
    "stylex_rowwise_sumsq": (ctypes.c_int, [_c_f, _c_f, _i64p, ctypes.c_void_p]),
    "stylex_reduce_chunks": (ctypes.c_int, [_i64p]),
    "stylex_act_bwd_reduce": (ctypes.c_int, [_c_f, _c_f, _c_f, _c_f, _i64p, ctypes.c_int, ctypes.c_int, ctypes.c_float,
                                             ctypes.c_int, ctypes.c_void_p]),
    "stylex_modconv_bwd_prep": (ctypes.c_int, [_c_f, _c_f, _c_f, ctypes.c_int64, _c_f, _c_f, _c_f, _c_f, _i64p,
                                               ctypes.c_int, ctypes.c_int, ctypes.c_int, ctypes.c_void_p]),
    "stylex_modconv_bwd_prep_scaled": (ctypes.c_int, [_c_f, _c_f, _c_f, ctypes.c_int64, _c_f, _c_f, _c_f, _c_f, _c_f, _i64p,
                                                      ctypes.c_int, ctypes.c_int, ctypes.c_int, ctypes.c_void_p]),
    "stylex_scale_reduce": (ctypes.c_int, [_c_f, _c_f, _c_f, _c_f, _c_f, _i64p, ctypes.c_int, ctypes.c_int,
                                           ctypes.c_void_p]),
    "stylex_pad_rgb8": (ctypes.c_int, [_c_f, _c_f, _i64p, _i64p, ctypes.c_int, ctypes.c_void_p]),
    "stylex_affine_act_nchw_fwd": (ctypes.c_int, [_c_f, _c_f, _c_f, _c_f, _c_f, ctypes.c_int64, ctypes.c_int64, ctypes.c_int64,
                                                  ctypes.c_int, ctypes.c_void_p]),
    "stylex_affine_act_nchw_bwd": (ctypes.c_int, [_c_f, _c_f, _c_f, _c_f, _c_f, ctypes.c_int64, ctypes.c_int64, ctypes.c_int64,
                                                  ctypes.c_int, ctypes.c_void_p]),
    "stylex_affine_relu_maxpool_fwd": (ctypes.c_int, [_c_f, _c_f, _c_f, _c_f, _c_f, ctypes.c_int64, ctypes.c_int64,
                                                      ctypes.c_int64, ctypes.c_int64, ctypes.c_void_p]),
    "stylex_affine_relu_maxpool_bwd": (ctypes.c_int, [_c_f, _c_f, _c_f, _c_f, ctypes.c_int64, ctypes.c_int64, ctypes.c_int64,
                                                      ctypes.c_int64, ctypes.c_void_p]),
    "stylex_lpips_tap_nhwc_fwd": (ctypes.c_int, [_c_f, _c_f, _c_f, _c_f, _c_f, _c_f, ctypes.c_int64, ctypes.c_int64, ctypes.c_int64,
                                                 ctypes.c_int64, ctypes.c_void_p]),
    "stylex_lpips_tap_nhwc_bwd": (ctypes.c_int, [_c_f, _c_f, _c_f, _c_f, _c_f, _c_f, _c_f, _c_f, ctypes.c_int64, ctypes.c_int64,
                                                 ctypes.c_int64, ctypes.c_void_p]),
    "stylex_nchw_f32_to_nhwc_bf16": (ctypes.c_int, [_c_f, _c_f, ctypes.c_int64, ctypes.c_int64, ctypes.c_int64, ctypes.c_int,
                                                    ctypes.c_void_p]),
    "stylex_nhwc_bf16_to_nchw_f32": (ctypes.c_int, [_c_f, _c_f, _c_f, ctypes.c_int64, ctypes.c_int64, ctypes.c_int64, ctypes.c_void_p]),
    "stylex_resize_norm_fwd": (ctypes.c_int, [_c_f, _c_f, _c_f, _c_f, _i64p, _i64p, ctypes.c_void_p]),
    "stylex_resize_norm_bwd": (ctypes.c_int, [_c_f, _c_f, _c_f, _i64p, ctypes.c_void_p]),
    "stylex_relu_gate_add": (ctypes.c_int, [_c_f, _c_f, _c_f, _c_f, ctypes.c_int64, ctypes.c_void_p]),
    "stylex_maxpool3s2_nhwc_fwd": (ctypes.c_int, [_c_f, _c_f, _c_f, _i64p, ctypes.c_void_p]),
    "stylex_maxpool3s2_nhwc_bwd": (ctypes.c_int, [_c_f, _c_f, _c_f, _i64p, ctypes.c_void_p]),
    "stylex_conv_image_grad": (ctypes.c_int, [_c_f, _c_f, _c_f, _i64p, ctypes.c_void_p]),
    "stylex_lpips_tap_fwd": (ctypes.c_int, [_c_f, _c_f, _c_f, _c_f, _c_f, _c_f, ctypes.c_int64, ctypes.c_int64, ctypes.c_int64,
                                            ctypes.c_int64, ctypes.c_void_p]),
    "stylex_lpips_tap_bwd": (ctypes.c_int, [_c_f, _c_f, _c_f, _c_f, _c_f, _c_f, _c_f, _c_f, ctypes.c_int64, ctypes.c_int64,
                                            ctypes.c_int64, ctypes.c_void_p]),
    "stylex_weight_sumsq": (ctypes.c_int, [_c_f, _c_f, ctypes.c_int64, ctypes.c_int64, ctypes.c_int64, ctypes.c_void_p]),
    "stylex_modcoeff_fwd": (ctypes.c_int, [_c_f, _c_f, _c_f, _c_f, ctypes.c_int64, ctypes.c_int64, ctypes.c_int64,
                                           ctypes.c_float, ctypes.c_void_p]),
    "stylex_modcoeff_bwd": (ctypes.c_int, [_c_f, _c_f, _c_f, _c_f, _c_f, _c_f, _c_f, _c_f, ctypes.c_int64, ctypes.c_int64,
                                           ctypes.c_int64, ctypes.c_int64, ctypes.c_void_p]),
    "stylex_torgb_chunks": (ctypes.c_int, [_i64p]),
    "stylex_torgb_fwd": (ctypes.c_int, [_c_f, _c_f, _c_f, _c_f, _i64p, ctypes.c_void_p]),
    "stylex_torgb_bwd": (ctypes.c_int, [_c_f, _c_f, _c_f, _c_f, _c_f, _c_f, _i64p, ctypes.c_void_p]),
    "stylex_timing_enable": (ctypes.c_int, [ctypes.c_int]),
    "stylex_timing_pause": (ctypes.c_int, [ctypes.c_int]),
    "stylex_timing_layers": (ctypes.c_int, [_i64p, ctypes.POINTER(ctypes.c_double), ctypes.c_int64]),
    "stylex_timing_kernels": (ctypes.c_int, [ctypes.c_char_p, _i64p, ctypes.POINTER(ctypes.c_double), ctypes.c_int64]),
    "stylex_conv2d_s2d_res_supported": (ctypes.c_int, [_i64p, ctypes.c_int64, ctypes.c_int64]),
    "stylex_conv2d_s2d_res_fwd": (ctypes.c_int, [ctypes.c_void_p] * 6 + [_i64p, ctypes.c_int64, ctypes.c_int64, ctypes.c_float,
                                                  ctypes.c_void_p]),
    "stylex_adam_pack_tensor_blocks": (ctypes.c_int64, [ctypes.c_int64, ctypes.c_int32, ctypes.c_int32, ctypes.c_int32]),
    "stylex_adam_pack_step": (ctypes.c_int, [ctypes.c_void_p, ctypes.c_void_p, ctypes.c_int64, ctypes.c_void_p]),
    "stylex_hinge_fwd": (ctypes.c_int, [_c_f, _c_f, _c_f, ctypes.c_int64, ctypes.c_int, ctypes.c_void_p]),
    "stylex_hinge_bwd": (ctypes.c_int, [_c_f] * 5 + [ctypes.c_int64, ctypes.c_int, ctypes.c_void_p]),
    "stylex_pl_lengths_fwd": (ctypes.c_int, [_c_f, _c_f, _i64p, ctypes.c_void_p]),
    "stylex_pl_lengths_bwd": (ctypes.c_int, [_c_f] * 4 + [_i64p, ctypes.c_void_p]),
    "stylex_kl_logits_fwd": (ctypes.c_int, [_c_f, _c_f, _c_f, _i64p, ctypes.c_void_p]),
    "stylex_kl_logits_bwd": (ctypes.c_int, [_c_f] * 5 + [_i64p, ctypes.c_void_p]),
    "stylex_l1_mean_chunks": (ctypes.c_int64, [ctypes.c_int64]),
    "stylex_l1_mean_fwd": (ctypes.c_int, [_c_f] * 4 + [ctypes.c_int64, ctypes.c_int, ctypes.c_int, _i64p, _i64p, _i64p,
                                            ctypes.c_void_p]),
    "stylex_l1_mean_bwd": (ctypes.c_int, [_c_f] * 5 + [ctypes.c_int64, ctypes.c_int, ctypes.c_int, _i64p, _i64p, _i64p,
                                            ctypes.c_void_p]),
    "stylex_linattn_chunks": (ctypes.c_int, [_i64p]),
    "stylex_linattn_fwd": (ctypes.c_int, [_c_f, _c_f, _c_f, _i64p, _c_f, _c_f, _c_f, _c_f, _c_f, _i64p, ctypes.c_int,
                                          ctypes.c_void_p]),
    "stylex_linattn_bwd": (ctypes.c_int, [_c_f, _c_f, _c_f, _i64p] + [_c_f] * 8 + [_i64p, ctypes.c_int, ctypes.c_void_p]),
    "stylex_chan_norm_fwd": (ctypes.c_int, [_c_f] * 6 + [_i64p, ctypes.c_float, ctypes.c_int, ctypes.c_void_p]),
    "stylex_chan_norm_bwd_blocks": (ctypes.c_int, [_i64p]),
    "stylex_chan_norm_bwd": (ctypes.c_int, [_c_f] * 8 + [_i64p, ctypes.c_float, ctypes.c_int, ctypes.c_void_p]),
    "stylex_dwconv3x3_fwd": (ctypes.c_int, [_c_f, _c_f, _c_f, _i64p, ctypes.c_int, ctypes.c_void_p]),
    "stylex_dwconv3x3_wgrad_blocks": (ctypes.c_int, [_i64p]),
    "stylex_dwconv3x3_bwd_weight": (ctypes.c_int, [_c_f, _c_f, _c_f, _c_f, _i64p, ctypes.c_int, ctypes.c_void_p]),
# ... 475 lines not shown
        if hit is not None and hit[0] is not None:
            return hit[0]
    wp = torch.cat([w.detach(), w.new_zeros(w.shape[0], extra, w.shape[2], w.shape[3])], dim=1)
    if key is not None:
        _cache_put(key, w, wp, None)
    return wp


def pack_weight(w, want_fwd=True, want_bwd=False, precision=F32, scale=None, owner=None):
    lib = _ensure_device(w)
    own = w if owner is None else owner
    cacheable = isinstance(own, torch.nn.Parameter) and w.is_contiguous() and w.dtype == torch.float32
    key = None
    if cacheable:
        key = (own.data_ptr(), tuple(w.shape), precision, scale) if owner is None else \
            (own.data_ptr(), tuple(w.shape), precision, scale, "derived")
        hit = _cache_hit(key, own)
        if hit is not None and (hit[0] is not None or not want_fwd) and (hit[1] is not None or not want_bwd):
            return hit
        if scale is None:
            want_fwd = want_bwd = True
    w_param = own
    w = w.contiguous()
    if w.dtype != torch.float32:
        w = w.float()
    if scale is not None:
        w = w.detach() * scale
    n, c, kh, kw = w.shape
    dt = torch.float32 if precision == F32 else torch.bfloat16
    wf = _empty(n * kh * kw * c, dtype=dt, device=w.device) if want_fwd else None
    wb = _empty(n * kh * kw * c, dtype=dt, device=w.device) if want_bwd else None
    _check(lib.stylex_pack_weight(_ptr(w), _ptr(wf), _ptr(wb), _shape(n, c, kh, kw), precision, _stream()),
           "stylex_pack_weight")
    if key is not None:
        _cache_put(key, w_param, wf, wb,
                   recipe=(lambda p: pack_weight(p, want_fwd, want_bwd, precision, scale)) if owner is None else None)
    return wf, wb


def pack_weight_fwd_as_dgrad(w, precision):
    lib = _ensure_device(w)
    cacheable = isinstance(w, torch.nn.Parameter) and w.is_contiguous() and w.dtype == torch.float32
    key = None
    if cacheable:
        key = (w.data_ptr(), tuple(w.shape), precision, "fwd_as_dgrad")
        hit = _cache_hit(key, w)
        if hit is not None:
            return hit[0]
    wm = w.detach().float().flip(2, 3).contiguous()
    n, c, kh, kw = wm.shape
    dt = torch.float32 if precision == F32 else torch.bfloat16
    wf = _empty(n * kh * kw * c, dtype=dt, device=w.device)
    _check(lib.stylex_pack_weight(_ptr(wm), _ptr(wf), None, _shape(n, c, kh, kw), precision, _stream()), "stylex_pack_weight")
    if key is not None:
        _cache_put(key, w, wf, None, recipe=lambda p: pack_weight_fwd_as_dgrad(p, precision))
    return wf


def pack_weight_s2d(w, scale=None):
    lib = _ensure_device(w)
    key = None
    if isinstance(w, torch.nn.Parameter) and w.is_contiguous() and w.dtype == torch.float32:
        key = (w.data_ptr(), tuple(w.shape), "s2d", scale)
        hit = _cache_hit(key, w)
        if hit is not None:
            return hit
    wc = w.contiguous().float()
    if scale is not None:
        wc = wc.detach() * scale
    n, c, kh, kw = wc.shape
    assert kh == 3 and kw == 3
    wf = _empty(n * 36 * c, dtype=torch.bfloat16, device=w.device)
    wb = _empty(n * 36 * c, dtype=torch.bfloat16, device=w.device)
    _check(lib.stylex_pack_weight_s2d(_ptr(wc), _ptr(wf), _ptr(wb), _shape(n, c, 3, 3), _stream()),
           "stylex_pack_weight_s2d")
    if key is not None:
        _cache_put(key, w, wf, wb, recipe=lambda p: pack_weight_s2d(p, scale))
    return wf, wb


_S2D_WGRAD_OK = {}


def conv2d_bwd_weight_s2d(x2, dy, w_shape, precision, out_scale=1.0, accumulate_into=None):
    lib = _ensure_device(x2)
    n, c = int(w_shape[0]), int(w_shape[1])
    ws2 = (n, 4 * c, 3, 3)
    sh = conv_shape(x2.shape, ws2, 1, 1)
    key = (tuple(sh), precision)
    ok = _S2D_WGRAD_OK.get(key)
    if ok is None:
        ok = _S2D_WGRAD_OK[key] = bool(precision == BF16_ACT and
                                       lib.stylex_conv2d_bwd_weight_s2d_supported(_shape(*sh), c, precision))
    if ok and os.environ.get("STYLEX_WGRAD_PIPE", "1") != "0" and x2.data_ptr() % 16 == 0 and dy.data_ptr() % 16 == 0:
        adt = act_dtype(precision)
        assert is_cl(x2) and is_cl(dy) and x2.dtype == adt and dy.dtype == adt, (x2.dtype, dy.dtype, adt)
        shp = _shape(*sh)
        nbytes = lib.stylex_conv2d_bwd_weight_workspace_bytes(shp)
        ws = _empty(max(nbytes // 4, 1), dtype=torch.float32, device=x2.device)
        dw = accumulate_into if accumulate_into is not None else _empty((n, c, 3, 3), dtype=torch.float32, device=x2.device)
        assert tuple(dw.shape) == (n, c, 3, 3) and (isinstance(dw, RawGrad) or (dw.dtype == torch.float32 and dw.is_contiguous()))
        _check(lib.stylex_conv2d_bwd_weight_s2d(_ptr(x2), _ptr(dy), _ptr(dw), _ptr(ws), nbytes, shp, c, float(out_scale),
                                                int(accumulate_into is not None), precision, _stream()),
               "stylex_conv2d_bwd_weight_s2d")
        return None if isinstance(dw, RawGrad) else dw
    dw = fold_weight_grad_s2d(conv2d_bwd_weight(x2, dy, ws2, 1, 1, precision, s2d_c=c), (n, c, 3, 3))
    if out_scale != 1.0:
        dw.mul_(out_scale)
    if isinstance(accumulate_into, RawGrad):
        return dw
    if accumulate_into is not None:
        return accumulate_into.add_(dw)
    return dw


def fold_weight_grad_s2d(dw2, w_shape):
    lib = _ensure_device(dw2)
    n, c = w_shape[0], w_shape[1]
    dw = _empty(tuple(w_shape), dtype=torch.float32, device=dw2.device)
    _check(lib.stylex_fold_weight_grad_s2d(_ptr(dw2.contiguous()), _ptr(dw), _shape(n, c, 3, 3), _stream()),
           "stylex_fold_weight_grad_s2d")
    return dw


def _split_workspace(lib, shp, which, precision, like):
    nbytes = lib.stylex_conv2d_workspace_bytes(shp, which, precision)
    if nbytes <= 0:
        return None, 0
    return _empty(nbytes // 4, dtype=torch.float32, device=like.device), nbytes


_MASK_OK = {}


def conv_mask_supported(sh, which, flags, precision):
    key = (tuple(sh), which, flags, precision)
    hit = _MASK_OK.get(key)
    if hit is None:
        hit = _MASK_OK[key] = bool(load_library().stylex_conv_mask_supported(_shape(*sh), which, flags, precision))
    return hit


_S2D_RES_OK = {}


def s2d_res_supported(xb_shape, n, s2d_c, res_c):
    key = (tuple(xb_shape), n, s2d_c, res_c)
    hit = _S2D_RES_OK.get(key)
    if hit is None:
        sh = conv_shape(xb_shape, (n, xb_shape[1], 3, 3), 1, 1)
        hit = _S2D_RES_OK[key] = bool(load_library().stylex_conv2d_s2d_res_supported(_shape(*sh), s2d_c, res_c))
    return hit


def conv2d_s2d_res_fwd(xb, wf2, xs, w_res_mat, bias, n, s2d_c, scale):
    lib = _ensure_device(xb)
    assert is_cl(xb) and is_cl(xs) and xb.dtype == torch.bfloat16 and xs.dtype == torch.bfloat16
    assert xs.shape[0] == xb.shape[0] and xs.shape[2:] == xb.shape[2:] and w_res_mat.shape == (n, xs.shape[1])
    sh = conv_shape(xb.shape, (n, xb.shape[1], 3, 3), 1, 1)
    y = empty_cl((sh[0], n, sh[9], sh[10]), xb, torch.bfloat16)
    bias = _f32(bias)
    _check(lib.stylex_conv2d_s2d_res_fwd(_ptr(xb), _ptr(wf2), _ptr(xs), _ptr(w_res_mat), _ptr(bias), _ptr(y), _shape(*sh),
                                         int(s2d_c), int(xs.shape[1]), float(scale), _stream()), "stylex_conv2d_s2d_res_fwd")
    return y


def conv2d_fwd(x, w, stride, pad, precision, bias=None, lrelu=False, in_scale=None, out_scale=None, noise=None,
               noise_w=None, noise_b=None, residual=None, res_scale=1.0, packed=None, w_shape=None, s2d_c=0,
               noise_natural=False, want_mask=False):
    lib = _ensure_device(x)
    adt = act_dtype(precision)
    assert is_cl(x) and x.dtype == adt, (x.dtype, adt)
    sh = conv_shape(x.shape, w_shape if packed is not None else w.shape, stride, pad)
    wf = packed if packed is not None else pack_weight(w, True, False, precision)[0]
    y = empty_cl((sh[0], sh[4], sh[9], sh[10]), x, adt)
    flags = 0
    epi = ConvEpilogue()
    epi.s2d_c = int(s2d_c)
    keep = []
    if in_scale is not None:
        in_scale = _f32(in_scale)
        keep.append(in_scale)
        epi.in_scale = in_scale.data_ptr()
    if bias is not None:
        bias = _f32(bias)
        keep.append(bias)
        flags |= EPI_BIAS
        epi.bias = bias.data_ptr()
    if lrelu:
        flags |= EPI_RELU if lrelu == "relu" else EPI_LRELU
    if out_scale is not None:
        out_scale = _f32(out_scale)
        keep.append(out_scale)
        flags |= EPI_OSCALE
        epi.out_scale = out_scale.data_ptr()
    if noise is not None:
# ... 276 lines not shown
    hit = _VEC_CACHE.get(key)
    if hit is not None and hit[0] == stamp and all(r() is p for r, p in zip(hit[1], params)):
        if hit[3] is not None and hit[4] != _stream_id():
            cur = torch.cuda.current_stream()
            cur.wait_event(hit[3])
            hit[2].record_stream(cur)
        return hit[2]
    if len(_VEC_CACHE) > 4096:
        _VEC_CACHE.clear()
    v = fn(*[p.detach() for p in params])
    if all(isinstance(p, torch.nn.Parameter) for p in params) and not (v.is_cuda and torch.cuda.is_current_stream_capturing()):
        ev = None
        if v.is_cuda:
            ev = torch.cuda.Event()
            ev.record()
        _VEC_CACHE[key] = (stamp, tuple(weakref.ref(p) for p in params), v, ev, _stream_id() if v.is_cuda else None)
    return v


def conv1x1_gemm_fwd(x, w, bias, owner=None):
    assert is_cl(x) and x.dtype == torch.bfloat16
    b, c, h, wd = x.shape
    wm = _bf16_matrix(w, owner=owner)
    x2 = x.permute(0, 2, 3, 1).reshape(b * h * wd, c)
    y2 = torch.mm(x2, wm.t()) if bias is None else torch.addmm(cached_vector("bf16", lambda t: t.to(torch.bfloat16), bias), x2, wm.t())
    return y2.view(b, h, wd, wm.shape[0]).permute(0, 3, 1, 2)


def conv1x1_gemm_bwd_data(dy, w, scale=None, owner=None):
    assert is_cl(dy) and dy.dtype == torch.bfloat16
    b, n, h, wd = dy.shape
    wm = _bf16_matrix(w, scale, owner=owner)
    dx2 = torch.mm(dy.permute(0, 2, 3, 1).reshape(b * h * wd, n), wm)
    return dx2.view(b, h, wd, wm.shape[1]).permute(0, 3, 1, 2)


def weight_sumsq(w):
    lib = _ensure_device(w)
    cacheable = isinstance(w, torch.nn.Parameter) and w.is_contiguous() and w.dtype == torch.float32
    key = None
    if cacheable:
        key = (w.data_ptr(), tuple(w.shape), "wsq", None)
        hit = _cache_hit(key, w)
        if hit is not None and hit[0] is not None:
            return hit[0]
    w_param = w
    w = w.detach().contiguous().float()
    o, c = w.shape[0], w.shape[1]
    k = w.numel() // (o * c)
    wsq = _empty(o * c, dtype=torch.float32, device=w.device).view(o, c)
    _check(lib.stylex_weight_sumsq(_ptr(w), _ptr(wsq), o, c, k, _stream()), "stylex_weight_sumsq")
    if key is not None:
        _cache_put(key, w_param, wsq, None, recipe=weight_sumsq)
    return wsq


def modcoeff_fwd(style, wsq, eps):
    lib = _ensure_device(style)
    style = _f32(style)
    b, c = style.shape
    o = wsq.shape[0]
    s1 = _empty(b * c, dtype=torch.float32, device=style.device).view(b, c)
    d = _empty(b * o, dtype=torch.float32, device=style.device).view(b, o)
    _check(lib.stylex_modcoeff_fwd(_ptr(style), _ptr(wsq), _ptr(s1), _ptr(d), b, c, o, float(eps), _stream()),
           "stylex_modcoeff_fwd")
    return s1, d


def modcoeff_bwd(gd, d, s1, wsq, w, gs1, want_style, want_weight):
    lib = _ensure_device(gd)
    gd = _f32(gd)
    gs1 = _f32(gs1)
    b, c = s1.shape
    o = d.shape[1]
    wc = w.detach().contiguous().float()
    k = wc.numel() // (o * c)
    gstyle = _empty(b * c, dtype=torch.float32, device=gd.device).view(b, c) if want_style else None
    gw = _empty(wc.numel(), dtype=torch.float32, device=gd.device).view(wc.shape) if want_weight else None
    _check(lib.stylex_modcoeff_bwd(_ptr(gd), _ptr(d), _ptr(s1), _ptr(wsq), _ptr(wc), _ptr(gs1), _ptr(gstyle), _ptr(gw), b, c,
                                   o, k, _stream()), "stylex_modcoeff_bwd")
    return gstyle, gw


def conv2d_bwd_weight(x, dy, w_shape, stride, pad, precision, x_scale=None, dy_scale=None, s2d_c=0, want_bias_sum=False,
                      out_scale=1.0, accumulate_into=None, accumulate_bias_into=None):
    lib = _ensure_device(x)
    adt = act_dtype(precision)
    assert is_cl(x) and is_cl(dy) and x.dtype == adt and dy.dtype == adt, (x.dtype, dy.dtype, adt)
    sh = conv_shape(x.shape, w_shape, stride, pad)
    shp = _shape(*sh)
    nbytes = lib.stylex_conv2d_bwd_weight_workspace_bytes(shp)
    if nbytes < 0:
        raise StylexHipError("bad wgrad shape %r" % (sh,))
    ws = _empty(max(nbytes // 4, 1), dtype=torch.float32, device=x.device)
    x_scale, dy_scale = _f32(x_scale), _f32(dy_scale)
    if out_scale != 1.0 or accumulate_into is not None:
        acc = accumulate_into is not None
        dw = accumulate_into if acc else _empty(tuple(w_shape), dtype=torch.float32, device=x.device)
        raw = isinstance(dw, RawGrad)
        assert tuple(dw.shape) == tuple(w_shape) and (raw or (dw.dtype == torch.float32 and dw.is_contiguous()))
        db, written = None, ctypes.c_int(0)
        if want_bias_sum:
            db = accumulate_bias_into if (acc and accumulate_bias_into is not None) else None
            if acc and db is None:
                return conv2d_bwd_weight(x, dy, w_shape, stride, pad, precision, x_scale, dy_scale, s2d_c, False, out_scale,
                                         accumulate_into), None
            if db is None:
                db = _empty(w_shape[0], dtype=torch.float32, device=x.device)
        _check(lib.stylex_conv2d_bwd_weight_ex(_ptr(x), _ptr(dy), _ptr(dw), _ptr(db), ctypes.byref(written), _ptr(ws), nbytes, shp,
                                               _ptr(x_scale), _ptr(dy_scale), int(s2d_c), float(out_scale), int(acc), precision,
                                               _stream()), "stylex_conv2d_bwd_weight_ex")
        dw = None if raw else dw
        if want_bias_sum:
            if not written.value:
                return dw, None
            return dw, (True if isinstance(db, RawGrad) else db)
        return dw
    dw = _empty(tuple(w_shape), dtype=torch.float32, device=x.device)
    if want_bias_sum:
        db = _empty(w_shape[0], dtype=torch.float32, device=x.device)
        written = ctypes.c_int(0)
        _check(lib.stylex_conv2d_bwd_weight_bias(_ptr(x), _ptr(dy), _ptr(dw), _ptr(db), ctypes.byref(written), _ptr(ws), nbytes,
                                                 shp, _ptr(x_scale), _ptr(dy_scale), int(s2d_c), precision, _stream()),
               "stylex_conv2d_bwd_weight_bias")
        return dw, (db if written.value else None)
    _check(lib.stylex_conv2d_bwd_weight(_ptr(x), _ptr(dy), _ptr(dw), _ptr(ws), nbytes, shp, _ptr(x_scale),
                                        _ptr(dy_scale), int(s2d_c), precision, _stream()), "stylex_conv2d_bwd_weight")
    return dw


def _ew(fn_name, x, out_shape, in_shape_for_kernel):
    lib = _ensure_device(x)
    assert is_cl(x) and x.dtype in (torch.float32, torch.bfloat16)
    y = empty_cl(out_shape, x)
    b, c, h, w = in_shape_for_kernel
    _check(getattr(lib, fn_name)(_ptr(x), _ptr(y), _shape(b, h, w, c), _adt(x), _stream()), fn_name)
    return y


def upsample2x_fwd(x):
    b, c, h, w = x.shape
    return _ew("stylex_upsample2x_bilinear_fwd", x, (b, c, 2 * h, 2 * w), (b, c, h, w))


def upsample2x_bwd(dy):
    b, c, h2, w2 = dy.shape
    return _ew("stylex_upsample2x_bilinear_bwd", dy, (b, c, h2 // 2, w2 // 2), (b, c, h2 // 2, w2 // 2))


def rgb_up_blur_add_fwd(rgb, prev=None):
    lib = _ensure_device(rgb)
    assert is_cl(rgb) and rgb.dtype in (torch.float32, torch.bfloat16)
    assert prev is None or (is_cl(prev) and prev.dtype == rgb.dtype and prev.shape == rgb.shape)
    b, c, h, w = rgb.shape
    y = empty_cl((b, c, 2 * h, 2 * w), rgb)
    _check(lib.stylex_rgb_up_blur_add_fwd(_ptr(rgb), _ptr(prev), _ptr(y), _shape(b, h, w, c), _adt(rgb), _stream()),
           "stylex_rgb_up_blur_add_fwd")
    return y


def rgb_up_blur_add_bwd(dy):
    b, c, h2, w2 = dy.shape
    return _ew("stylex_rgb_up_blur_add_bwd", dy, (b, c, h2 // 2, w2 // 2), (b, c, h2 // 2, w2 // 2))


def blur3x3_fwd(x):
    return _ew("stylex_blur3x3_reflect_fwd", x, tuple(x.shape), tuple(x.shape))


def blur3x3_bwd(dy):
    return _ew("stylex_blur3x3_reflect_bwd", dy, tuple(dy.shape), tuple(dy.shape))


def blur3x3_s2d_fwd(x):
    lib = _ensure_device(x)
    assert is_cl(x)
    b, c, h, w = x.shape
    y = empty_cl((b, 4 * c, h // 2, w // 2), x)
    _check(lib.stylex_blur3x3_s2d_fwd(_ptr(x), _ptr(y), _shape(b, h, w, c), _adt(x), _stream()), "stylex_blur3x3_s2d_fwd")
    return y


def blur_mask_ok(shape, dtype):
    _, c, h, w = shape
    return dtype == torch.bfloat16 and c % 8 == 0 and h >= 8 and h % 2 == 0 and w % 2 == 0


def blur3x3_s2d_bwd(dy2, gate=None, slope=0.2, gate_mask=None):
    lib = _ensure_device(dy2)
    assert is_cl(dy2)
    b, c4, h2, w2 = dy2.shape
    dx = empty_cl((b, c4 // 4, 2 * h2, 2 * w2), dy2)
    shp = _shape(b, 2 * h2, 2 * w2, c4 // 4)
# ... 472 lines not shown
```

### explaining-in-style-reproducibility-study_amd/stylex/ops.py

```python
import math

import os

import torch
from contextlib import nullcontext as _nullcontext
import torch.nn.functional as F

import hip_backend as hb

_PRECISION = hb.F32


_NAMES = {"fp32": hb.F32, "f32": hb.F32, "bf16": hb.BF16_ACT, "bf16_f32act": hb.BF16}


def set_precision(name):
    global _PRECISION
    _PRECISION = _NAMES[name]


def get_precision():
    return {hb.F32: "fp32", hb.BF16_ACT: "bf16", hb.BF16: "bf16_f32act"}[_PRECISION]


# ... 636 lines not shown
        res_gemm = _PRECISION == hb.BF16_ACT and os.environ.get("STYLEX_RES_GEMM", "1") != "0"
        conv_res = (lambda t: hb.conv1x1_gemm_fwd(t, wrp if cin == 3 else w_res, b_res,
                                                  owner=w_res if cin == 3 else None)) if res_gemm else (
            lambda t: hb.conv2d_fwd(t, wrp, 1, 0, _PRECISION, bias=b_res))
        n2_, h2_, w2_ = w2.shape[0], x.shape[2], x.shape[3]
        fold_res = (bool(downsample) and _PRECISION == hb.BF16_ACT and res_gemm and h2_ % 2 == 0 and w2_ % 2 == 0
                    and n2_ % 64 == 0 and x.shape[1] % 8 == 0 and os.environ.get("STYLEX_RES_FOLD", "1") != "0"
                    and hb.s2d_res_supported((x.shape[0], 4 * n2_, h2_ // 2, w2_ // 2), w_res.shape[0], n2_, x.shape[1]))
        res = None
        if fold_res:
            xs = hb.subsample2_fwd(x)
            side = None
        elif side is None:
            xs = hb.subsample2_fwd(x) if downsample else x
            res = conv_res(xs)
        else:
            main = torch.cuda.current_stream()
            side.wait_stream(main)
            with torch.cuda.stream(side):
                xs = hb.subsample2_fwd(x) if downsample else x
                res = conv_res(xs)
            x.record_stream(side)
        n2, h2, wd2 = w2.shape[0], x.shape[2], x.shape[3]
        s2d_next = bool(downsample) and (_PRECISION != hb.F32 and n2 % 64 == 0 and h2 % 2 == 0 and wd2 % 2 == 0
                                         and wd2 // 2 >= 16 and h2 // 2 >= 16)
        use_m = (_PRECISION == hb.BF16_ACT and os.environ.get("STYLEX_GATE_MASK", "1") != "0"
                 and h2 * wd2 >= int(os.environ.get("STYLEX_GATE_MASK_MIN_PIXELS", 128 * 128)))
        pk1 = dict(packed=hb.pack_weight(w1p, True, False, _PRECISION, owner=w1)[0], w_shape=tuple(w1p.shape)) \
            if (cin == 3 and w1p is not w1 and isinstance(w1, torch.nn.Parameter)) else {}
        y1, m1 = hb.conv2d_fwd(x, w1p, 1, 1, _PRECISION, bias=b1, lrelu=True, want_mask=True, **pk1) if use_m else (
            hb.conv2d_fwd(x, w1p, 1, 1, _PRECISION, bias=b1, lrelu=True, **pk1), None)
        want_m2 = use_m and s2d_next and hb.blur_mask_ok((x.shape[0], n2, h2, wd2), x.dtype)
        y2, m2 = hb.conv2d_fwd(y1, w2, 1, 1, _PRECISION, bias=b2, lrelu=True, want_mask=True) if want_m2 else (
            hb.conv2d_fwd(y1, w2, 1, 1, _PRECISION, bias=b2, lrelu=True), None)
        s2d, xb = False, None
        def join():
            if side is not None:
                torch.cuda.current_stream().wait_stream(side)
                res.record_stream(torch.cuda.current_stream())
                xs.record_stream(torch.cuda.current_stream())

        if downsample:
            n, h, w = y2.shape[1], y2.shape[2], y2.shape[3]
            s2d = (_PRECISION != hb.F32 and n % 64 == 0 and h % 2 == 0 and w % 2 == 0 and w // 2 >= 16 and h // 2 >= 16)
            if s2d:
                xb = hb.blur3x3_s2d_fwd(y2)
                join()
                wf2, _ = hb.pack_weight_s2d(w3)
                if fold_res:
                    wm = hb._bf16_matrix(wrp if cin == 3 else w_res, owner=w_res if cin == 3 else None)
                    bsum = hb.cached_vector("sum32", lambda a, b: a.float() + b.float(), b3, b_res)
                    out = hb.conv2d_s2d_res_fwd(xb, wf2, xs, wm, bsum, w3.shape[0], n, c)
                else:
                    out = hb.conv2d_fwd(xb, None, 1, 1, _PRECISION, bias=b3, residual=res, res_scale=c, packed=wf2,
                                        w_shape=(w3.shape[0], 4 * n, 3, 3), s2d_c=n)
            else:
                xb = hb.blur3x3_fwd(y2)
                join()
                out = hb.conv2d_fwd(xb, w3, 2, 1, _PRECISION, bias=b3, residual=res, res_scale=c)
        else:
            join()
            out = (y2 + res) * c
        assert m2 is None or s2d
        ctx.save_for_backward(x, xs if downsample else None, y1, y2 if m2 is None else None, xb, w_res, w1, w2, w3, m1, m2)
        ctx.y2_shape = tuple(y2.shape)
        ctx.cfg = (bool(downsample), s2d, cin, c)
        return out

    @staticmethod
    @torch.autograd.function.once_differentiable
    def backward(ctx, g_out):
        x, xs, y1, y2, xb, w_res, w1, w2, w3, m1, m2 = ctx.saved_tensors
        downsample, s2d, cin, c = ctx.cfg
        if xs is None:
            xs = x
        need = ctx.needs_input_grad
        want_x = need[0]
        want_b = need[2] or need[4] or need[6] or need[8]
        want_w = need[1] or need[3] or need[5] or need[7]
        g_out = _cl(g_out)
        prec = _PRECISION
        gw_res = gb_res = gw1 = gb1 = gw2 = gb2 = gw3 = gb3 = gx = None
        alg = downsample and prec != hb.F32
        if alg:
            gz3 = g_out
            gsum3 = _channel_sum(g_out, c) if want_b else None
        elif _reducible(g_out.shape[1]):
            gz3, gsum3 = hb.act_bwd_reduce(g_out, None, False, c, want_dx=True, want_sum=want_b)
        else:
            gz3 = g_out * c
            gsum3 = gz3.sum(dim=(0, 2, 3), dtype=torch.float32) if want_b else None
        wsc = c if alg else 1.0
        gb_res = gsum3
        if cin == 3:
            extra = x.shape[1] - 3
            w1p, wrp = hb.pad_in_channels(w1, extra), hb.pad_in_channels(w_res, extra)
        else:
            w1p, wrp = w1, w_res
        side_bwd, side_out, main = _fork_side(g_out), None, torch.cuda.current_stream() if g_out.is_cuda else None
        res_gemm = prec == hb.BF16_ACT and os.environ.get("STYLEX_RES_GEMM", "1") != "0"

        def res_dgrad():
            if res_gemm:
                return hb.conv1x1_gemm_bwd_data(gz3, wrp if cin == 3 else w_res, scale=c if alg else None,
                                                owner=w_res if cin == 3 else None)
            wbr = hb.pack_weight(wrp, False, True, prec, scale=c)[1] if alg else None
            return hb.conv2d_bwd_data(gz3, wrp, tuple(xs.shape), 1, 0, prec, packed=wbr, w_shape=tuple(wrp.shape))

        a_res = _gacc_get(w_res) if (want_w and cin != 3) else None
        if side_bwd is not None:
            side_bwd.wait_stream(main)
            with torch.cuda.stream(side_bwd):
                s_gw = s_gx = None
                if want_w:
                    s_gw = hb.conv2d_bwd_weight(xs, gz3, tuple(wrp.shape), 1, 0, prec, out_scale=wsc, accumulate_into=a_res)
                if want_x:
                    s_gx = res_dgrad()
                side_out = (s_gw, s_gx)
            gz3.record_stream(side_bwd)
            xs.record_stream(side_bwd)
        if downsample:
            gb3 = gsum3
            n = ctx.y2_shape[1]
            if s2d:
                _, wb2 = hb.pack_weight_s2d(w3, scale=c if alg else None)
                gxb = hb.conv2d_bwd_data(gz3, None, tuple(xb.shape), 1, 1, prec, packed=wb2, w_shape=(w3.shape[0], 4 * n, 3, 3),
                                         s2d_c=n)
                if want_w:
                    a3 = _gacc_get(w3)
                    gw3 = hb.conv2d_bwd_weight_s2d(xb, gz3, tuple(w3.shape), prec, out_scale=wsc, accumulate_into=a3)
                    if a3 is None and need[7]:
                        _gacc_put(w3, gw3)
                gz2 = hb.blur3x3_s2d_bwd(gxb, gate=y2, gate_mask=m2)
            else:
                wb3 = hb.pack_weight(w3, False, True, prec, scale=c)[1] if alg else None
                gxb = hb.conv2d_bwd_data(gz3, w3, tuple(xb.shape), 2, 1, prec, packed=wb3, w_shape=tuple(w3.shape))
                if want_w:
                    a3 = _gacc_get(w3)
                    gw3 = hb.conv2d_bwd_weight(xb, gz3, tuple(w3.shape), 2, 1, prec, out_scale=wsc, accumulate_into=a3)
                    if a3 is None and need[7]:
                        _gacc_put(w3, gw3)
                gz2 = hb.blur3x3_bwd_gate(gxb, y2)
        else:
            gz2 = hb.bias_act_bwd(gz3, y2)
        fuse_b = want_b and want_w and os.environ.get("STYLEX_WGRAD_BIAS", "1") != "0"
        acc_b2 = False
        if want_w:
            a2w, a2b = _gacc_get(w2), _gacc_get(w2, "b")
            gw2 = hb.conv2d_bwd_weight(y1, gz2, tuple(w2.shape), 1, 1, prec, want_bias_sum=fuse_b, accumulate_into=a2w,
                                       accumulate_bias_into=a2b if a2w is not None else None)
            if fuse_b:
                gw2, gb2 = gw2
                if gb2 is True:
                    gb2, acc_b2 = None, True
            if a2w is None:
                if need[5]:
                    _gacc_put(w2, gw2)
                if need[6]:
                    _gacc_put(w2, gb2, "b")
        if want_b and gb2 is None and not acc_b2:
            gb2 = _channel_sum(gz2)
        gz1 = hb.conv2d_bwd_data(gz2, w2, tuple(y1.shape), 1, 1, prec, gate=y1, gate_mask=m1)
        if getattr(ctx, "keep_gz", False):
            ctx.gz = (gz3, gz2, gz1, alg)
        gxs = None
        acc_b1 = False
        if want_w:
            a1w = _gacc_get(w1) if cin != 3 else None
            a1b = _gacc_get(w1, "b") if a1w is not None else None
            gw1 = hb.conv2d_bwd_weight(x, gz1, tuple(w1p.shape), 1, 1, prec, want_bias_sum=fuse_b, accumulate_into=a1w,
                                       accumulate_bias_into=a1b)
            if fuse_b:
                gw1, gb1 = gw1
                if gb1 is True:
                    gb1, acc_b1 = None, True
            if a1w is None and cin != 3:
                if need[3]:
                    _gacc_put(w1, gw1)
                if need[4]:
                    _gacc_put(w1, gb1, "b")
        if want_b and gb1 is None and not acc_b1:
            gb1 = _channel_sum(gz1)
        if want_x:
            pk1 = dict(packed=hb.pack_weight(w1p, False, True, prec, owner=w1)[1], w_shape=tuple(w1p.shape)) \
                if (cin == 3 and isinstance(w1, torch.nn.Parameter)) else {}
            gx = hb.conv2d_bwd_data(gz1, w1p, tuple(x.shape), 1, 1, prec, **pk1)
        if side_bwd is not None:
            gw_res, gxs = side_out
            main.wait_stream(side_bwd)
            for t in (gw_res, gxs):
                if t is not None:
                    t.record_stream(main)
        else:
            if want_w:
                gw_res = hb.conv2d_bwd_weight(xs, gz3, tuple(wrp.shape), 1, 0, prec, out_scale=wsc, accumulate_into=a_res)
            if want_x:
                gxs = res_dgrad()
        if want_w and a_res is None and cin != 3 and need[1]:
            _gacc_put(w_res, gw_res)
        if want_w and cin == 3:
            gw1, gw_res = gw1[:, :3].contiguous(), gw_res[:, :3].contiguous()
        if want_x:
            if downsample:
                hb.add_at_even_(gx, gxs)
            else:
                gx += gxs
            if cin == 3:
                gx = gx[:, :3]
        return (gx, gw_res if need[1] else None, gb_res if need[2] else None, gw1 if need[3] else None,
                gb1 if need[4] else None, gw2 if need[5] else None, gb2 if need[6] else None,
                gw3 if need[7] else None, gb3 if need[8] else None, None)


_GACC = {}
_GACC_TASK = [-2]
_GACC_ON = os.environ.get("STYLEX_GRAD_ACC", "1") != "0"
_GACC_STREAMS = set()
_GACC_WAITED = {}
_GACC_SEQ = [0]


def _gacc_join():
    if _GACC_STREAMS:
        cur = torch.cuda.current_stream()
        for st in _GACC_STREAMS:
            if st != cur:
                cur.wait_stream(st)
        _GACC_STREAMS.clear()


def _gacc_get(w, tag=""):
    if not _GACC_ON or not w.is_cuda:
        return None
    task = torch._C._current_graph_task_id()
    if task < 0:
        return None
    if task != _GACC_TASK[0]:
        _GACC.clear()
        _GACC_STREAMS.clear()
        _GACC_WAITED.clear()
        _GACC_TASK[0] = task
    slot = _GACC.get((w.data_ptr(), tag))
    if slot is not None and not slot.alive():
        del _GACC[(w.data_ptr(), tag)]
        return None
    if slot is not None:
        cur = torch.cuda.current_stream()
        if slot.stream != cur:
            key = (cur, slot.stream)
            if _GACC_WAITED.get(key, 0) <= slot.seq:
                cur.wait_stream(slot.stream)
                _GACC_WAITED[key] = _GACC_SEQ[0]
            if not _GACC_STREAMS:
                torch.autograd.Variable._execution_engine.queue_callback(_gacc_join)
            _GACC_STREAMS.add(cur)
    return slot


def _gacc_put(w, g, tag=""):
    if _GACC_ON and g is not None and w.is_cuda and torch._C._current_graph_task_id() == _GACC_TASK[0] and g.is_contiguous():
        slot = _GACC[(w.data_ptr(), tag)] = hb.RawGrad(g)
        slot.seq = _GACC_SEQ[0]
        _GACC_SEQ[0] += 1


def _channel_sum(t, scale=1.0):
    if _reducible(t.shape[1]):
        return hb.act_bwd_reduce(t, None, False, scale, want_dx=False, want_sum=True)[1]
    r = t.sum(dim=(0, 2, 3), dtype=torch.float32)
    return r if scale == 1.0 else r * scale




def _pad_rgb(x, weight):
    n_out = weight.shape[0]
    if weight.shape[1] == 3:
        extra = 5 if x.dtype == torch.bfloat16 else 1
        x = torch.cat([x, x.new_zeros(x.shape[0], extra, x.shape[2], x.shape[3])], dim=1)
        weight = torch.cat([weight, weight.new_zeros(weight.shape[0], extra, weight.shape[2], weight.shape[3])], dim=1)
# ... 443 lines not shown
```

### include/stylex_hip.h

```cpp
#ifndef STYLEX_HIP_H
#define STYLEX_HIP_H

#include <stdint.h>

#ifdef __cplusplus
extern "C" {
#endif

#define STYLEX_F32 0
#define STYLEX_BF16 1
#define STYLEX_BF16_ACT 2

#define STYLEX_EINVAL (-1)
#define STYLEX_EWORKSPACE (-2)

#define STYLEX_CONV_NSHAPE 11

#define STYLEX_EPI_BIAS 1
#define STYLEX_EPI_LRELU 2
#define STYLEX_EPI_OSCALE 4
#define STYLEX_EPI_NOISE 8
#define STYLEX_EPI_RESIDUAL 16
#define STYLEX_EPI_RELU 32
#define STYLEX_EPI_NOISE_NAT 128
#define STYLEX_EPI_MASK_OUT 256
#define STYLEX_EPI_GATE_MASK 512
#define STYLEX_EPI_GATE 64

int stylex_init(int device);
const char* stylex_version(void);

int stylex_pack_weight(const float* w_oihw, void* w_fwd, void* w_bwd, const int64_t* shape, int precision,
                       void* stream);

typedef struct {
    const float* in_scale;
    const float* bias;
    const float* out_scale;
    const float* noise;
    int64_t noise_stride;
    const float* noise_w;
    const float* noise_b;
    const void* residual;
    float res_scale;
    int32_t s2d_c;
    void* mask;
} stylex_conv_epilogue;

int stylex_conv_mask_supported(const int64_t* shape, int which, int flags, int precision);

int64_t stylex_conv2d_workspace_bytes(const int64_t* shape, int which, int precision);

int stylex_conv2d_fwd(const void* x, const void* w_fwd, void* y, const int64_t* shape, int flags,
                      const stylex_conv_epilogue* epi, int precision, void* workspace, int64_t workspace_bytes,
                      void* stream);

int stylex_conv2d_s2d_res_supported(const int64_t* shape, int64_t s2d_c, int64_t res_c);
int stylex_conv2d_s2d_res_fwd(const void* x_s2d, const void* w_fwd_s2d, const void* x_res, const void* w_res, const float* bias,
                              void* y, const int64_t* shape, int64_t s2d_c, int64_t res_c, float scale, void* stream);

int stylex_conv2d_bwd_data(const void* dy, const void* w_bwd, void* dx, const int64_t* shape, int flags,
                           const stylex_conv_epilogue* epi, int precision, void* workspace, int64_t workspace_bytes,
                           void* stream);

int64_t stylex_conv2d_bwd_weight_workspace_bytes(const int64_t* shape);
int stylex_conv2d_bwd_weight(const void* x, const void* dy, float* dw, void* workspace, int64_t workspace_bytes,
                             const int64_t* shape, const float* x_scale, const float* dy_scale, int s2d_c,
                             int precision, void* stream);
int stylex_conv2d_bwd_weight_bias(const void* x, const void* dy, float* dw, float* db, int* db_written, void* workspace,
                                  int64_t workspace_bytes, const int64_t* shape, const float* x_scale,
                                  const float* dy_scale, int s2d_c, int precision, void* stream);
int stylex_conv2d_bwd_weight_ex(const void* x, const void* dy, float* dw, float* db, int* db_written, void* workspace,
                                int64_t workspace_bytes, const int64_t* shape, const float* x_scale, const float* dy_scale,
                                int s2d_c, float out_scale, int accumulate, int precision, void* stream);

int stylex_upsample2x_bilinear_fwd(const void* x, void* y, const int64_t* shape, int act_dtype, void* stream);
int stylex_upsample2x_bilinear_bwd(const void* dy, void* dx, const int64_t* shape, int act_dtype, void* stream);

int stylex_blur3x3_reflect_fwd(const void* x, void* y, const int64_t* shape, int act_dtype, void* stream);
int stylex_blur3x3_reflect_bwd(const void* dy, void* dx, const int64_t* shape, int act_dtype, void* stream);

int stylex_rgb_up_blur_add_fwd(const void* rgb, const void* prev, void* out, const int64_t* shape, int act_dtype,
                               void* stream);
int stylex_rgb_up_blur_add_bwd(const void* dy, void* dx, const int64_t* shape, int act_dtype, void* stream);

int stylex_blur3x3_s2d_fwd(const void* x, void* y_s2d, const int64_t* shape, int act_dtype, void* stream);
int stylex_blur3x3_s2d_bwd(const void* dy_s2d, void* dx, const int64_t* shape, int act_dtype, void* stream);
int stylex_blur3x3_reflect_bwd_gate(const void* dy, const void* gate, float slope, void* dx, const int64_t* shape,
                                    int act_dtype, void* stream);
int stylex_blur3x3_s2d_bwd_gate(const void* dy_s2d, const void* gate, float slope, void* dx, const int64_t* shape,
                                int act_dtype, void* stream);
int stylex_blur3x3_s2d_bwd_gate_mask(const void* dy_s2d, const void* mask, float slope, void* dx, const int64_t* shape,
                                     int act_dtype, void* stream);
int stylex_add_at_even(const void* src, void* dst, const int64_t* shape, int act_dtype, void* stream);

int stylex_subsample2_fwd(const void* x, void* y, const int64_t* shape, int act_dtype, void* stream);
int stylex_subsample2_bwd(const void* dy, void* dx, const int64_t* shape, int act_dtype, void* stream);
int stylex_pack_weight_s2d(const float* w_oihw, void* w_fwd, void* w_bwd, const int64_t* shape, void* stream);
int stylex_fold_weight_grad_s2d(const float* dw_s2d, float* dw_oihw, const int64_t* shape, void* stream);
int stylex_conv2d_bwd_weight_s2d_supported(const int64_t* shape, int s2d_c, int precision);
int stylex_conv2d_bwd_weight_s2d(const void* x2, const void* dy, float* dw_oihw, void* workspace, int64_t workspace_bytes,
                                 const int64_t* shape, int s2d_c, float out_scale, int accumulate, int precision, void* stream);

int stylex_bias_act_fwd(const void* x, const float* bias, const float* noise, int64_t noise_stride,
                        const float* noise_w, const float* noise_b, void* y, const int64_t* shape, int act_dtype,
                        void* stream);
int stylex_bias_act_bwd(const void* dy, const void* y, void* dx, const int64_t* shape, int act_dtype, void* stream);

int stylex_rowwise_sumsq(const float* x, float* out, const int64_t* shape, void* stream);

int stylex_pad_rgb8(const void* x, void* y, const int64_t* shape_bhw, const int64_t* strides_bchw, int x_is_bf16, void* stream);

int stylex_affine_act_nchw_fwd(const float* x, const float* scale, const float* shift, const float* residual, float* y, int64_t B,
                               int64_t C, int64_t HW, int relu, void* stream);
int stylex_affine_act_nchw_bwd(const float* gy, const float* y, const float* scale, float* gx, float* gres, int64_t B, int64_t C,
                               int64_t HW, int relu, void* stream);
int stylex_affine_relu_maxpool_fwd(const float* x, const float* scale, const float* shift, float* y, unsigned char* idx, int64_t B,
                                   int64_t C, int64_t H, int64_t W, void* stream);
int stylex_affine_relu_maxpool_bwd(const float* gy, const unsigned char* idx, const float* scale, float* gx, int64_t B, int64_t C,
                                   int64_t H, int64_t W, void* stream);

int stylex_resize_norm_fwd(const float* x, float* y, const float* mean, const float* stdv, const int64_t* sh, const int64_t* strides,
                           void* stream);
int stylex_resize_norm_bwd(const float* gy, float* gx, const float* stdv, const int64_t* sh, void* stream);

int stylex_relu_gate_add(const void* a, const void* b, const void* y, void* out, int64_t numel, void* stream);
int stylex_nchw_f32_to_nhwc_bf16(const float* x, void* y, int64_t B, int64_t C, int64_t HW, int relu, void* stream);
int stylex_nhwc_bf16_to_nchw_f32(const void* g, const void* gate, float* gx, int64_t B, int64_t C, int64_t HW, void* stream);

int stylex_maxpool3s2_nhwc_fwd(const void* x, void* y, void* idx, const int64_t* sh, void* stream);
int stylex_maxpool3s2_nhwc_bwd(const void* gy, const void* idx, void* gx, const int64_t* sh, void* stream);

int stylex_conv_image_grad(const float* dy, const float* w, float* dx, const int64_t* sh, void* stream);

int stylex_lpips_tap_fwd(const float* f0, const float* f1, const float* lin, float* partial, float* r0, float* r1, int64_t B,
                         int64_t C, int64_t HW, int64_t partial_stride, void* stream);
int stylex_lpips_tap_bwd(const float* f0, const float* f1, const float* lin, const float* r0, const float* r1, const float* gout,
                         float* g0, float* g1, int64_t B, int64_t C, int64_t HW, void* stream);

int stylex_lpips_tap_nhwc_fwd(const void* f0, const void* f1, const float* lin, float* partial, float* r0, float* r1, int64_t B,
                              int64_t C, int64_t HW, int64_t partial_stride, void* stream);
int stylex_lpips_tap_nhwc_bwd(const void* f0, const void* f1, const float* lin, const float* r0, const float* r1, const float* gout,
                              void* g0, void* g1, int64_t B, int64_t C, int64_t HW, void* stream);

int stylex_weight_sumsq(const float* w, float* wsq, int64_t O, int64_t C, int64_t K, void* stream);
int stylex_modcoeff_fwd(const float* style, const float* wsq, float* s1, float* d, int64_t B, int64_t C, int64_t O,
                        float eps, void* stream);
int stylex_modcoeff_bwd(const float* gd, const float* d, const float* s1, const float* wsq, const float* w,
                        const float* gs1, float* gstyle, float* gw, int64_t B, int64_t C, int64_t O, int64_t K,
                        void* stream);

int stylex_reduce_chunks(const int64_t* shape);
int stylex_act_bwd_reduce(const void* dy, const void* y, void* dx, float* partial, const int64_t* shape, int nchunks,
                          int lrelu, float scale, int act_dtype, void* stream);
int stylex_modconv_bwd_prep(const void* gy, const void* y, const float* noise, int64_t noise_stride,
                            const float* noise_w, const float* noise_b, void* gz, float* partial,
                            const int64_t* shape, int nchunks, int lrelu, int act_dtype, void* stream);
int stylex_modconv_bwd_prep_scaled(const void* gy, const void* y, const float* noise, int64_t noise_stride,
                                   const float* noise_w, const float* noise_b, const float* gz_scale, void* gz,
                                   float* partial, const int64_t* shape, int nchunks, int lrelu, int act_dtype,
                                   void* stream);
int stylex_scale_reduce(const void* x, const void* t, const float* s, void* gx, float* partial, const int64_t* shape,
                        int nchunks, int act_dtype, void* stream);

int stylex_torgb_chunks(const int64_t* shape);
int stylex_torgb_fwd(const void* x, const float* s1, const float* w, void* y, const int64_t* shape, void* stream);
int stylex_torgb_bwd(const void* x, const void* gy, const float* s1, const float* w, void* gx, float* partial,
                     const int64_t* shape, void* stream);

int stylex_timing_enable(int on);
int stylex_timing_pause(int on);
int stylex_timing_report(int kernel_class, int64_t* launches, double* total_ms, double* total_flops,
                         double* total_bytes);
int stylex_timing_layers(int64_t* meta, double* vals, int64_t cap);
int stylex_timing_kernels(char* names, int64_t* meta, double* vals, int64_t cap);

#define STYLEX_ADAM_COPY_PACK 0
#define STYLEX_ADAM_COPY_PACK_S2D 1
#define STYLEX_ADAM_COPY_SUMSQ 2
typedef struct {
    float* p;
    const float* g;
    float* m;
    float* v;
    const float* step;
// ... 58 lines not shown
```

Measured before the change: 994.6 images/sec.

## Fuse bias-gradient channel sums into space-to-depth and transposed wgrad kernels

Extends the fused bias-sum path, where an extra MFMA against a ones vector accumulates dy column sums, to the space-to-depth wgrad pipe kernel and the transposed wgrad kernels. The wgrad reduce kernel then folds the bias partials, and a new fresh-bias flag lets the bias be written fresh while the weight gradient still accumulates. In the discriminator's downsampling residual block this replaces a separate channel-sum pass over g_out. The cost is an extra MFMA per step for the bias-owning waves plus more template instantiations and flag plumbing.

Measured after the change: 1011 images/sec (median of 4 runs). 1.02x the previous value.

```diff
diff --git a/explaining-in-style-reproducibility-study_amd/csrc/conv_igemm.hip b/explaining-in-style-reproducibility-study_amd/csrc/conv_igemm.hip
--- a/explaining-in-style-reproducibility-study_amd/csrc/conv_igemm.hip
+++ b/explaining-in-style-reproducibility-study_amd/csrc/conv_igemm.hip
@@ -650,7 +650,7 @@
                                                            const float* __restrict__ bias_part, float* db, float scale, int accum) {
     __shared__ float tile[256 * 9];
     if ((int)blockIdx.x >= main_blocks) {
-        bias_reduce_block(bias_part, db, N, splits, blockIdx.x - main_blocks, scale, accum);
+        bias_reduce_block(bias_part, db, N, splits, blockIdx.x - main_blocks, scale, (accum & STYLEX_WG_DB_FRESH) ? 0 : accum);
         return;
     }
     const long total = (long)N * C * T;
@@ -712,7 +712,7 @@
     static_assert(PP * G == 256, "one thread per (pair, slice group)");
     __shared__ float red[G][PP][9];
     if ((int)blockIdx.x >= main_blocks) {
-        bias_reduce_block(bias_part, db, N, splits, blockIdx.x - main_blocks, scale, accum);
+        bias_reduce_block(bias_part, db, N, splits, blockIdx.x - main_blocks, scale, (accum & STYLEX_WG_DB_FRESH) ? 0 : accum);
         return;
     }
     const long total = (long)N * C * T;
@@ -1097,10 +1097,16 @@
         p.bias_partial = nullptr;
     }
     if (precision == STYLEX_BF16 && stylex_wgrad_tr_applicable(p)) {
-        int ts = 0;
-        int rc = stylex_launch_wgrad_tr(p, partial, s, &ts);
+        int ts = 0, mode, bias_done = 0;
+        long len;
+        stylex_wgrad_tr_plan(p, &mode, &ts, &len);
+        p.bias_partial = db ? partial + (long)ts * p.N * p.KH * p.KW * p.Ck : nullptr;
+        int rc = stylex_launch_wgrad_tr(p, partial, s, &ts, &bias_done);
         if (rc) return rc;
-        launch_wgrad_reduce(partial, dw_oihw, p.N, p.Ck, p.KH * p.KW, ts, s, wg_out_of(p));
+        const bool with_db = db && bias_done;
+        launch_wgrad_reduce(partial, dw_oihw, p.N, p.Ck, p.KH * p.KW, ts, s, wg_out_of(p), with_db ? p.bias_partial : nullptr,
+                            with_db ? db : nullptr);
+        if (with_db && db_done) *db_done = 1;
         return (int)hipGetLastError();
     }
     int tn, tc, splits;
@@ -1129,11 +1135,17 @@
     return (int)hipGetLastError();
 }
 
-int stylex_launch_wgrad_s2d_folded(ConvKParams p, float* partial, float* dw_oihw, hipStream_t s) {
-    int slices = 0;
-    int rc = stylex_launch_wgrad_pipe(p, partial, s, &slices, nullptr);
+int stylex_launch_wgrad_s2d_folded(ConvKParams p, float* partial, float* dw_oihw, hipStream_t s, float* db, int* db_done) {
+    int slices = 0, tps, blocks, bias_done = 0;
+    if (db_done) *db_done = 0;
+    stylex_wgrad_pipe_plan(p, &slices, &tps, &blocks);
+    p.bias_partial = db ? partial + (long)slices * p.N * 9 * p.s2d_c : nullptr;
+    int rc = stylex_launch_wgrad_pipe(p, partial, s, &slices, &bias_done);
     if (rc) return rc == STYLEX_NOT_APPLICABLE ? STYLEX_EINVAL : rc;
-    launch_wgrad_reduce(partial, dw_oihw, p.N, p.s2d_c, 9, slices, s, wg_out_of(p));
+    const bool with_db = db && bias_done;
+    launch_wgrad_reduce(partial, dw_oihw, p.N, p.s2d_c, 9, slices, s, wg_out_of(p), with_db ? p.bias_partial : nullptr,
+                        with_db ? db : nullptr);
+    if (with_db && db_done) *db_done = 1;
     return (int)hipGetLastError();
 }
 
diff --git a/explaining-in-style-reproducibility-study_amd/csrc/conv_wgrad_pipe.hip b/explaining-in-style-reproducibility-study_amd/csrc/conv_wgrad_pipe.hip
--- a/explaining-in-style-reproducibility-study_amd/csrc/conv_wgrad_pipe.hip
+++ b/explaining-in-style-reproducibility-study_amd/csrc/conv_wgrad_pipe.hip
@@ -153,7 +153,6 @@
     static_assert(NSTEP % 2 == 0, "the operand ping-pong restarts at parity 0 every stage");
     static_assert(NSLOT <= 2 * (NSTEP - 1), "at most two DMA pieces per step");
     static_assert(XA <= DA, "issue order inside a stage: the one-ahead stream first");
-    static_assert(!(S2D && BIAS), "the space-to-depth path has no bias sums");
     extern __shared__ __attribute__((aligned(16))) char smem[];
     const int tid = threadIdx.x, lane = tid & 63;
     const int wave = __builtin_amdgcn_readfirstlane(tid >> 6);
@@ -406,6 +405,10 @@
         const int Co = p.s2d_c, sy = sub >> 1, sx = sub & 1;
         float* outf = p.y + (long)split * N * 9 * Co;
         const int cl = c0 - sub * Co + cblk * 32 + lj;
+        if (do_bias && lj == 0) {
+#pragma unroll
+            for (int r = 0; r < 16; ++r) p.bias_partial[(long)split * N + nbase + (r & 3) + 8 * (r >> 2) + 4 * lh] = accb[r];
+        }
 #pragma unroll
         for (int t2 = 0; t2 < 5; ++t2) {
             if (t2 == 2) continue;
@@ -439,17 +442,21 @@
 }
 
 template <int NP64, int TW>
-int launch_wg_s2d(const ConvKParams& p, const WgArgs& wa, int blocks, hipStream_t s) {
+int launch_wg_s2d(const ConvKParams& p, const WgArgs& wa, int blocks, bool bias, hipStream_t s) {
     using Cfg = WgCfg<NP64, TW>;
     static int attr_state = 0;
     if (attr_state == 0) {
         hipError_t e = hipFuncSetAttribute(reinterpret_cast<const void*>(conv3x3_wgrad_pipe_kernel<NP64, TW, false, true>),
                                            hipFuncAttributeMaxDynamicSharedMemorySize, Cfg::SMEM);
+        if (e == hipSuccess)
+            e = hipFuncSetAttribute(reinterpret_cast<const void*>(conv3x3_wgrad_pipe_kernel<NP64, TW, true, true>),
+                                    hipFuncAttributeMaxDynamicSharedMemorySize, Cfg::SMEM);
         attr_state = e == hipSuccess ? 1 : -1;
     }
     if (attr_state < 0) return STYLEX_NOT_APPLICABLE;
-    stylex_note_kernel("conv3x3_wgrad_pipe_kernel<%d, %d, false, true>", NP64, TW);
-    hipLaunchKernelGGL((conv3x3_wgrad_pipe_kernel<NP64, TW, false, true>), dim3(blocks), dim3(512), Cfg::SMEM, s, p, wa);
+    stylex_note_kernel("conv3x3_wgrad_pipe_kernel<%d, %d, %s, true>", NP64, TW, bias ? "true" : "false");
+    if (bias) hipLaunchKernelGGL((conv3x3_wgrad_pipe_kernel<NP64, TW, true, true>), dim3(blocks), dim3(512), Cfg::SMEM, s, p, wa);
+    else hipLaunchKernelGGL((conv3x3_wgrad_pipe_kernel<NP64, TW, false, true>), dim3(blocks), dim3(512), Cfg::SMEM, s, p, wa);
     return (int)hipGetLastError();
 }
 
@@ -550,10 +557,10 @@
     p.y = partial;
     *slices_out = slices;
     if (p.s2d_c) {
-        if (bias_done) *bias_done = 0;
-        p.bias_partial = nullptr;
-        if (np64 == 2) return tw == 32 ? launch_wg_s2d<2, 32>(p, wa, blocks, s) : launch_wg_s2d<2, 16>(p, wa, blocks, s);
-        return tw == 32 ? launch_wg_s2d<1, 32>(p, wa, blocks, s) : launch_wg_s2d<1, 16>(p, wa, blocks, s);
+        const bool sb = p.bias_partial != nullptr;
+        if (bias_done) *bias_done = sb ? 1 : 0;
+        if (np64 == 2) return tw == 32 ? launch_wg_s2d<2, 32>(p, wa, blocks, sb, s) : launch_wg_s2d<2, 16>(p, wa, blocks, sb, s);
+        return tw == 32 ? launch_wg_s2d<1, 32>(p, wa, blocks, sb, s) : launch_wg_s2d<1, 16>(p, wa, blocks, sb, s);
     }
     const bool bias = p.bias_partial != nullptr;
     if (bias_done) *bias_done = bias ? 1 : 0;
diff --git a/explaining-in-style-reproducibility-study_amd/csrc/conv_wgrad_tr.hip b/explaining-in-style-reproducibility-study_amd/csrc/conv_wgrad_tr.hip
--- a/explaining-in-style-reproducibility-study_amd/csrc/conv_wgrad_tr.hip
+++ b/explaining-in-style-reproducibility-study_amd/csrc/conv_wgrad_tr.hip
@@ -131,6 +131,7 @@
                     if (p.a_scale) v = scaled(v, p.a_scale + (long)b * C + c);
                 }
             }
+            if (C8 && q == T && p.bias_partial) v = make_uint4(0x3F803F80u, 0x3F803F80u, 0x3F803F80u, 0x3F803F80u);
             rb[j] = v;
         }
     };
@@ -197,6 +198,15 @@
 #pragma unroll
     for (int j = 0; j < TC_; ++j) {
         const int cj = c0 + (wc * TC_ + j) * 32 + lj;
+        if (C8 && p.bias_partial && cj == T * 8) {
+#pragma unroll
+            for (int i = 0; i < TN_; ++i)
+#pragma unroll
+                for (int r = 0; r < 16; ++r) {
+                    const int n = n0 + (wn * TN_ + i) * 32 + (r & 3) + 8 * (r >> 2) + 4 * lh;
+                    if (n < N) p.bias_partial[(long)split * N + n] = acc[i][j][r];
+                }
+        }
         if (C8 ? (cj >= T * 8) : (cj >= C)) continue;
 #pragma unroll
         for (int i = 0; i < TN_; ++i)
@@ -241,6 +251,7 @@
     return r;
 }
 
+template <bool BIAS>
 __global__ __launch_bounds__(512, 1) void conv_wgrad_tr_dma_kernel(ConvKParams p) {
     extern __shared__ __attribute__((aligned(16))) char smem[];
     const int tid = threadIdx.x, lane = tid & 63;
@@ -304,11 +315,15 @@
     };
 
     const int wn = wave >> 1, wc = wave & 1;
-    f32x16 acc[2];
+    f32x16 acc[2], accb;
 #pragma unroll
     for (int j = 0; j < 2; ++j)
 #pragma unroll
         for (int e = 0; e < 16; ++e) acc[j][e] = 0.f;
+#pragma unroll
+    for (int e = 0; e < 16; ++e) accb[e] = 0.f;
+    const bool do_bias = BIAS && p.bias_partial != nullptr && tap == 0 && c0 == 0 && wc == 0;
+    const bf16x8 ones = {0x3F80, 0x3F80, 0x3F80, 0x3F80, 0x3F80, 0x3F80, 0x3F80, 0x3F80};
     const int i16 = lane & 15, g = lane >> 4;
     const int lane_off = ((g >> 1) * 8 + (i16 >> 2)) * 64 + ((g & 1) * 16 + (i16 & 3) * 4) * 2;
     const int lds0 = (int)(unsigned)(uintptr_t)(lds_void_ptr)smem;
@@ -339,11 +354,20 @@
             const bf16x8 av = cat8(o[ks & 1].a[0], o[ks & 1].a[1]);
             acc[0] = __builtin_amdgcn_mfma_f32_32x32x16_bf16(av, cat8(o[ks & 1].b[0][0], o[ks & 1].b[0][1]), acc[0], 0, 0, 0);
             acc[1] = __builtin_amdgcn_mfma_f32_32x32x16_bf16(av, cat8(o[ks & 1].b[1][0], o[ks & 1].b[1][1]), acc[1], 0, 0, 0);
+            if constexpr (BIAS) {
+                if (do_bias) accb = __builtin_amdgcn_mfma_f32_32x32x16_bf16(av, ones, accb, 0, 0, 0);
+            }
         }
     }
 
     const int lj = lane & 31, lh = lane >> 5;
     float* out = p.y + (long)split * N * T * C;
+    if constexpr (BIAS) {
+        if (do_bias && lj == 0) {
+#pragma unroll
+            for (int r = 0; r < 16; ++r) p.bias_partial[(long)split * N + n0 + wn * 32 + (r & 3) + 8 * (r >> 2) + 4 * lh] = accb[r];
+        }
+    }
 #pragma unroll
     for (int j = 0; j < 2; ++j) {
         const int cj = c0 + (wc * 2 + j) * 32 + lj;
@@ -421,7 +445,7 @@
     *split_len = len;
 }
 
-int stylex_launch_wgrad_tr(ConvKParams p, float* partial, hipStream_t s, int* splits_out) {
+int stylex_launch_wgrad_tr(ConvKParams p, float* partial, hipStream_t s, int* splits_out, int* bias_done) {
     int mode, splits;
     long len;
     stylex_wgrad_tr_plan(p, &mode, &splits, &len);
@@ -429,19 +453,36 @@
     p.y = partial;
     *splits_out = splits;
     const int T = p.KH * p.KW;
-    if (mode == 2) return launch_tr<1, 2, true>(p, ((p.N + 63) / 64) * splits, s);
+    if (bias_done) *bias_done = 0;
+    if (p.a2_scale) p.bias_partial = nullptr;
+    if (mode == 2) {
+        if (T >= 16) p.bias_partial = nullptr;
+        if (bias_done && p.bias_partial) *bias_done = 1;
+        return launch_tr<1, 2, true>(p, ((p.N + 63) / 64) * splits, s);
+    }
     if (mode == 0 && tr_dma_applicable(p)) {
         static bool attr_done = false;
         if (!attr_done) {
-            hipError_t e = hipFuncSetAttribute(reinterpret_cast<const void*>(conv_wgrad_tr_dma_kernel),
+            hipError_t e = hipFuncSetAttribute(reinterpret_cast<const void*>(conv_wgrad_tr_dma_kernel<false>),
                                                hipFuncAttributeMaxDynamicSharedMemorySize, DSTAGES * DSTAGE_BYTES);
+            if (e == hipSuccess)
+                e = hipFuncSetAttribute(reinterpret_cast<const void*>(conv_wgrad_tr_dma_kernel<true>),
+                                        hipFuncAttributeMaxDynamicSharedMemorySize, DSTAGES * DSTAGE_BYTES);
             if (e != hipSuccess) return (int)e;
             attr_done = true;
         }
-        stylex_note_kernel("conv_wgrad_tr_dma_kernel");
-        hipLaunchKernelGGL(conv_wgrad_tr_dma_kernel, dim3((p.N / 128) * (p.Ck / 128) * T * splits), dim3(512), DSTAGES * DSTAGE_BYTES, s, p);
+        const dim3 grid((p.N / 128) * (p.Ck / 128) * T * splits);
+        if (p.bias_partial) {
+            if (bias_done) *bias_done = 1;
+            stylex_note_kernel("conv_wgrad_tr_dma_kernel<true>");
+            hipLaunchKernelGGL(conv_wgrad_tr_dma_kernel<true>, grid, dim3(512), DSTAGES * DSTAGE_BYTES, s, p);
+        } else {
+            stylex_note_kernel("conv_wgrad_tr_dma_kernel<false>");
+            hipLaunchKernelGGL(conv_wgrad_tr_dma_kernel<false>, grid, dim3(512), DSTAGES * DSTAGE_BYTES, s, p);
+        }
         return (int)hipGetLastError();
     }
+    p.bias_partial = nullptr;
     if (mode == 0) return launch_tr<2, 2, false>(p, ((p.N + 127) / 128) * ((p.Ck + 127) / 128) * T * splits, s);
     return launch_tr<1, 1, false>(p, ((p.N + 63) / 64) * ((p.Ck + 63) / 64) * T * splits, s);
 }
diff --git a/explaining-in-style-reproducibility-study_amd/csrc/stylex_capi.hip b/explaining-in-style-reproducibility-study_amd/csrc/stylex_capi.hip
--- a/explaining-in-style-reproducibility-study_amd/csrc/stylex_capi.hip
+++ b/explaining-in-style-reproducibility-study_amd/csrc/stylex_capi.hip
@@ -434,6 +434,12 @@
     p.M = p.B * p.Ho * p.Wo;
 }
 
+static int wg_flags(int accumulate) {
+    if (!accumulate) return 0;
+    return (accumulate & STYLEX_WG_DB_FRESH) && (accumulate & STYLEX_WG_ACCUMULATE) ? (STYLEX_WG_ACCUMULATE | STYLEX_WG_DB_FRESH)
+                                                                                    : STYLEX_WG_ACCUMULATE;
+}
+
 int64_t stylex_conv2d_bwd_weight_workspace_bytes(const int64_t* sh) {
     if (!conv_shape_ok(sh)) return STYLEX_EINVAL;
     ConvKParams p;
@@ -500,7 +506,7 @@
     if (p.act_bf16) precision = STYLEX_BF16;
     p.s2d_c = s2d_c;
     p.wg_scale = out_scale;
-    p.wg_accumulate = accumulate ? 1 : 0;
+    p.wg_accumulate = wg_flags(accumulate);
     if (s2d_c && (p.Ck != 4 * s2d_c || s2d_c % 64 || p.KH != 3 || p.stride != 1)) return STYLEX_EINVAL;
     double flops = 2.0 * p.M * (double)p.N * p.Ck * p.KH * p.KW / (s2d_c ? 4.0 : 1.0);
     ScopedTimer tm(2, flops, conv_bytes(sh, p.act_bf16 ? STYLEX_BF16_ACT : precision, true), (hipStream_t)stream, sh, s2d_c);
@@ -518,6 +524,15 @@
 
 int stylex_conv2d_bwd_weight_s2d(const void* x2, const void* dy, float* dw, void* workspace, int64_t workspace_bytes,
                                  const int64_t* sh, int s2d_c, float out_scale, int accumulate, int precision, void* stream) {
+    return stylex_conv2d_bwd_weight_s2d_bias(x2, dy, dw, nullptr, nullptr, workspace, workspace_bytes, sh, s2d_c, out_scale,
+                                             accumulate, precision, stream);
+}
+
+int stylex_conv2d_bwd_weight_s2d_bias(const void* x2, const void* dy, float* dw, float* db, int* db_written, void* workspace,
+                                      int64_t workspace_bytes, const int64_t* sh, int s2d_c, float out_scale, int accumulate,
+                                      int precision, void* stream) {
+    if (db_written) *db_written = 0;
+    if (db && !db_written) return STYLEX_EINVAL;
     if (!x2 || !dy || !dw || !workspace || !conv_shape_ok(sh) || precision != STYLEX_BF16_ACT || s2d_c <= 0) return STYLEX_EINVAL;
     if (workspace_bytes < stylex_conv2d_bwd_weight_workspace_bytes(sh)) return STYLEX_EWORKSPACE;
     ConvKParams p;
@@ -527,11 +542,11 @@
     p.act_bf16 = 1;
     p.s2d_c = s2d_c;
     p.wg_scale = out_scale;
-    p.wg_accumulate = accumulate ? 1 : 0;
+    p.wg_accumulate = wg_flags(accumulate);
     if (!stylex_wgrad_pipe_applicable(p)) return STYLEX_EINVAL;
     double flops = 2.0 * p.M * (double)p.N * p.Ck * 9 / 4.0;
     ScopedTimer tm(2, flops, conv_bytes(sh, STYLEX_BF16_ACT, true), (hipStream_t)stream, sh, s2d_c);
-    return stylex_launch_wgrad_s2d_folded(p, (float*)workspace, dw, (hipStream_t)stream);
+    return stylex_launch_wgrad_s2d_folded(p, (float*)workspace, dw, (hipStream_t)stream, db, db_written);
 }
 
 int stylex_pack_weight_s2d(const float* w, void* wf, void* wb, const int64_t* sh, void* stream) {
diff --git a/explaining-in-style-reproducibility-study_amd/csrc/stylex_internal.h b/explaining-in-style-reproducibility-study_amd/csrc/stylex_internal.h
--- a/explaining-in-style-reproducibility-study_amd/csrc/stylex_internal.h
+++ b/explaining-in-style-reproducibility-study_amd/csrc/stylex_internal.h
@@ -95,11 +95,12 @@
 bool stylex_wgrad_pipe_applicable(const ConvKParams& p);
 void stylex_wgrad_pipe_plan(const ConvKParams& p, int* slices, int* tiles_per_split, int* blocks);
 int stylex_launch_wgrad_pipe(ConvKParams p, float* partial, hipStream_t s, int* slices_out, int* bias_done = nullptr);
-int stylex_launch_wgrad_s2d_folded(ConvKParams p, float* partial, float* dw_oihw, hipStream_t s);
+int stylex_launch_wgrad_s2d_folded(ConvKParams p, float* partial, float* dw_oihw, hipStream_t s, float* db = nullptr,
+                                   int* db_done = nullptr);
 
 bool stylex_wgrad_tr_applicable(const ConvKParams& p);
 void stylex_wgrad_tr_plan(const ConvKParams& p, int* mode, int* splits, long* split_len);
-int stylex_launch_wgrad_tr(ConvKParams p, float* partial, hipStream_t s, int* splits_out);
+int stylex_launch_wgrad_tr(ConvKParams p, float* partial, hipStream_t s, int* splits_out, int* bias_done = nullptr);
 
 __host__ __device__ inline unsigned stylex_s2d_tap_mask(int s) {
     const int sy = s >> 1, sx = s & 1;
diff --git a/explaining-in-style-reproducibility-study_amd/stylex/hip_backend.py b/explaining-in-style-reproducibility-study_amd/stylex/hip_backend.py
--- a/explaining-in-style-reproducibility-study_amd/stylex/hip_backend.py
+++ b/explaining-in-style-reproducibility-study_amd/stylex/hip_backend.py
@@ -69,6 +69,9 @@
     "stylex_conv2d_bwd_weight_s2d_supported": (ctypes.c_int, [_i64p, ctypes.c_int, ctypes.c_int]),
     "stylex_conv2d_bwd_weight_s2d": (ctypes.c_int, [ctypes.c_void_p, ctypes.c_void_p, _c_f, ctypes.c_void_p, ctypes.c_int64, _i64p,
                                                     ctypes.c_int, ctypes.c_float, ctypes.c_int, ctypes.c_int, ctypes.c_void_p]),
+    "stylex_conv2d_bwd_weight_s2d_bias": (ctypes.c_int, [ctypes.c_void_p, ctypes.c_void_p, _c_f, _c_f, ctypes.POINTER(ctypes.c_int),
+                                                         ctypes.c_void_p, ctypes.c_int64, _i64p, ctypes.c_int, ctypes.c_float,
+                                                         ctypes.c_int, ctypes.c_int, ctypes.c_void_p]),
     "stylex_upsample2x_bilinear_fwd": (ctypes.c_int, [_c_f, _c_f, _i64p, ctypes.c_int, ctypes.c_void_p]),
     "stylex_upsample2x_bilinear_bwd": (ctypes.c_int, [_c_f, _c_f, _i64p, ctypes.c_int, ctypes.c_void_p]),
     "stylex_rgb_up_blur_add_fwd": (ctypes.c_int, [_c_f, _c_f, _c_f, _i64p, ctypes.c_int, ctypes.c_void_p]),
@@ -710,7 +713,7 @@
 _S2D_WGRAD_OK = {}
 
 
-def conv2d_bwd_weight_s2d(x2, dy, w_shape, precision, out_scale=1.0, accumulate_into=None):
+def conv2d_bwd_weight_s2d(x2, dy, w_shape, precision, out_scale=1.0, accumulate_into=None, want_bias_sum=False):
     lib = _ensure_device(x2)
     n, c = int(w_shape[0]), int(w_shape[1])
     ws2 = (n, 4 * c, 3, 3)
@@ -728,18 +731,24 @@
         ws = _empty(max(nbytes // 4, 1), dtype=torch.float32, device=x2.device)
         dw = accumulate_into if accumulate_into is not None else _empty((n, c, 3, 3), dtype=torch.float32, device=x2.device)
         assert tuple(dw.shape) == (n, c, 3, 3) and (isinstance(dw, RawGrad) or (dw.dtype == torch.float32 and dw.is_contiguous()))
+        if want_bias_sum and os.environ.get("STYLEX_WGRAD_BIAS", "1") != "0":
+            db, written = _empty(n, dtype=torch.float32, device=x2.device), ctypes.c_int(0)
+            _check(lib.stylex_conv2d_bwd_weight_s2d_bias(_ptr(x2), _ptr(dy), _ptr(dw), _ptr(db), ctypes.byref(written), _ptr(ws),
+                                                         nbytes, shp, c, float(out_scale),
+                                                         WG_ACCUMULATE | WG_DB_FRESH if accumulate_into is not None else 0,
+                                                         precision, _stream()), "stylex_conv2d_bwd_weight_s2d_bias")
+            return (None if isinstance(dw, RawGrad) else dw), (db if written.value else None)
         _check(lib.stylex_conv2d_bwd_weight_s2d(_ptr(x2), _ptr(dy), _ptr(dw), _ptr(ws), nbytes, shp, c, float(out_scale),
                                                 int(accumulate_into is not None), precision, _stream()),
                "stylex_conv2d_bwd_weight_s2d")
-        return None if isinstance(dw, RawGrad) else dw
+        dw = None if isinstance(dw, RawGrad) else dw
+        return (dw, None) if want_bias_sum else dw
     dw = fold_weight_grad_s2d(conv2d_bwd_weight(x2, dy, ws2, 1, 1, precision, s2d_c=c), (n, c, 3, 3))
     if out_scale != 1.0:
         dw.mul_(out_scale)
-    if isinstance(accumulate_into, RawGrad):
-        return dw
-    if accumulate_into is not None:
-        return accumulate_into.add_(dw)
-    return dw
+    if accumulate_into is not None and not isinstance(accumulate_into, RawGrad):
+        dw = accumulate_into.add_(dw)
+    return (dw, None) if want_bias_sum else dw
 
 
 def fold_weight_grad_s2d(dw2, w_shape):
@@ -1182,8 +1191,11 @@
     return gstyle, gw
 
 
+WG_ACCUMULATE, WG_DB_FRESH = 1, 2
+
+
 def conv2d_bwd_weight(x, dy, w_shape, stride, pad, precision, x_scale=None, dy_scale=None, s2d_c=0, want_bias_sum=False,
-                      out_scale=1.0, accumulate_into=None, accumulate_bias_into=None):
+                      out_scale=1.0, accumulate_into=None, accumulate_bias_into=None, fresh_bias=False):
     lib = _ensure_device(x)
     adt = act_dtype(precision)
     assert is_cl(x) and is_cl(dy) and x.dtype == adt and dy.dtype == adt, (x.dtype, dy.dtype, adt)
@@ -1201,14 +1213,15 @@
         assert tuple(dw.shape) == tuple(w_shape) and (raw or (dw.dtype == torch.float32 and dw.is_contiguous()))
         db, written = None, ctypes.c_int(0)
         if want_bias_sum:
-            db = accumulate_bias_into if (acc and accumulate_bias_into is not None) else None
-            if acc and db is None:
+            db = accumulate_bias_into if (acc and accumulate_bias_into is not None and not fresh_bias) else None
+            if acc and db is None and not fresh_bias:
                 return conv2d_bwd_weight(x, dy, w_shape, stride, pad, precision, x_scale, dy_scale, s2d_c, False, out_scale,
                                          accumulate_into), None
             if db is None:
                 db = _empty(w_shape[0], dtype=torch.float32, device=x.device)
+        flags = (WG_ACCUMULATE | WG_DB_FRESH if fresh_bias and want_bias_sum else WG_ACCUMULATE) if acc else 0
         _check(lib.stylex_conv2d_bwd_weight_ex(_ptr(x), _ptr(dy), _ptr(dw), _ptr(db), ctypes.byref(written), _ptr(ws), nbytes, shp,
-                                               _ptr(x_scale), _ptr(dy_scale), int(s2d_c), float(out_scale), int(acc), precision,
+                                               _ptr(x_scale), _ptr(dy_scale), int(s2d_c), float(out_scale), flags, precision,
                                                _stream()), "stylex_conv2d_bwd_weight_ex")
         dw = None if raw else dw
         if want_bias_sum:
diff --git a/explaining-in-style-reproducibility-study_amd/stylex/ops.py b/explaining-in-style-reproducibility-study_amd/stylex/ops.py
--- a/explaining-in-style-reproducibility-study_amd/stylex/ops.py
+++ b/explaining-in-style-reproducibility-study_amd/stylex/ops.py
@@ -742,16 +742,17 @@
         prec = _PRECISION
         gw_res = gb_res = gw1 = gb1 = gw2 = gb2 = gw3 = gb3 = gx = None
         alg = downsample and prec != hb.F32
+        fuse_b = want_b and want_w and os.environ.get("STYLEX_WGRAD_BIAS", "1") != "0"
         if alg:
             gz3 = g_out
-            gsum3 = _channel_sum(g_out, c) if want_b else None
+            gsum3 = None if fuse_b else (_channel_sum(g_out, c) if want_b else None)
         elif _reducible(g_out.shape[1]):
             gz3, gsum3 = hb.act_bwd_reduce(g_out, None, False, c, want_dx=True, want_sum=want_b)
         else:
             gz3 = g_out * c
             gsum3 = gz3.sum(dim=(0, 2, 3), dtype=torch.float32) if want_b else None
         wsc = c if alg else 1.0
-        gb_res = gsum3
+        take3 = alg and fuse_b
         if cin == 3:
             extra = x.shape[1] - 3
             w1p, wrp = hb.pad_in_channels(w1, extra), hb.pad_in_channels(w_res, extra)
@@ -780,7 +781,6 @@
             gz3.record_stream(side_bwd)
             xs.record_stream(side_bwd)
         if downsample:
-            gb3 = gsum3
             n = ctx.y2_shape[1]
             if s2d:
                 _, wb2 = hb.pack_weight_s2d(w3, scale=c if alg else None)
@@ -788,7 +788,10 @@
                                          s2d_c=n)
                 if want_w:
                     a3 = _gacc_get(w3)
-                    gw3 = hb.conv2d_bwd_weight_s2d(xb, gz3, tuple(w3.shape), prec, out_scale=wsc, accumulate_into=a3)
+                    gw3 = hb.conv2d_bwd_weight_s2d(xb, gz3, tuple(w3.shape), prec, out_scale=wsc, accumulate_into=a3,
+                                                   want_bias_sum=take3)
+                    if take3:
+                        gw3, gsum3 = gw3
                     if a3 is None and need[7]:
                         _gacc_put(w3, gw3)
                 gz2 = hb.blur3x3_s2d_bwd(gxb, gate=y2, gate_mask=m2)
@@ -797,13 +800,15 @@
                 gxb = hb.conv2d_bwd_data(gz3, w3, tuple(xb.shape), 2, 1, prec, packed=wb3, w_shape=tuple(w3.shape))
                 if want_w:
                     a3 = _gacc_get(w3)
-                    gw3 = hb.conv2d_bwd_weight(xb, gz3, tuple(w3.shape), 2, 1, prec, out_scale=wsc, accumulate_into=a3)
+                    gw3 = hb.conv2d_bwd_weight(xb, gz3, tuple(w3.shape), 2, 1, prec, out_scale=wsc, accumulate_into=a3,
+                                               want_bias_sum=take3, fresh_bias=True)
+                    if take3:
+                        gw3, gsum3 = gw3
                     if a3 is None and need[7]:
                         _gacc_put(w3, gw3)
                 gz2 = hb.blur3x3_bwd_gate(gxb, y2)
         else:
             gz2 = hb.bias_act_bwd(gz3, y2)
-        fuse_b = want_b and want_w and os.environ.get("STYLEX_WGRAD_BIAS", "1") != "0"
         acc_b2 = False
         if want_w:
             a2w, a2b = _gacc_get(w2), _gacc_get(w2, "b")
@@ -853,9 +858,18 @@
                     t.record_stream(main)
         else:
             if want_w:
-                gw_res = hb.conv2d_bwd_weight(xs, gz3, tuple(wrp.shape), 1, 0, prec, out_scale=wsc, accumulate_into=a_res)
+                take_r = take3 and gsum3 is None
+                gw_res = hb.conv2d_bwd_weight(xs, gz3, tuple(wrp.shape), 1, 0, prec, out_scale=wsc, accumulate_into=a_res,
+                                              want_bias_sum=take_r, fresh_bias=True)
+                if take_r:
+                    gw_res, gsum3 = gw_res
             if want_x:
                 gxs = res_dgrad()
+        if alg and want_b and gsum3 is None:
+            gsum3 = _channel_sum(g_out, c)
+        gb_res = gsum3
+        if downsample:
+            gb3 = gsum3
         if want_w and a_res is None and cin != 3 and need[1]:
             _gacc_put(w_res, gw_res)
         if want_w and cin == 3:
diff --git a/include/stylex_hip.h b/include/stylex_hip.h
--- a/include/stylex_hip.h
+++ b/include/stylex_hip.h
@@ -70,6 +70,8 @@
 int stylex_conv2d_bwd_weight_bias(const void* x, const void* dy, float* dw, float* db, int* db_written, void* workspace,
                                   int64_t workspace_bytes, const int64_t* shape, const float* x_scale,
                                   const float* dy_scale, int s2d_c, int precision, void* stream);
+#define STYLEX_WG_ACCUMULATE 1
+#define STYLEX_WG_DB_FRESH 2
 int stylex_conv2d_bwd_weight_ex(const void* x, const void* dy, float* dw, float* db, int* db_written, void* workspace,
                                 int64_t workspace_bytes, const int64_t* shape, const float* x_scale, const float* dy_scale,
                                 int s2d_c, float out_scale, int accumulate, int precision, void* stream);
@@ -101,6 +103,9 @@
 int stylex_conv2d_bwd_weight_s2d_supported(const int64_t* shape, int s2d_c, int precision);
 int stylex_conv2d_bwd_weight_s2d(const void* x2, const void* dy, float* dw_oihw, void* workspace, int64_t workspace_bytes,
                                  const int64_t* shape, int s2d_c, float out_scale, int accumulate, int precision, void* stream);
+int stylex_conv2d_bwd_weight_s2d_bias(const void* x2, const void* dy, float* dw_oihw, float* db, int* db_written, void* workspace,
+                                      int64_t workspace_bytes, const int64_t* shape, int s2d_c, float out_scale, int accumulate,
+                                      int precision, void* stream);
 
 int stylex_bias_act_fwd(const void* x, const float* bias, const float* noise, int64_t noise_stride,
                         const float* noise_w, const float* noise_b, void* y, const int64_t* shape, int act_dtype,
```
